# adthoms/dcora

Hardware: AMD Instinct MI355X
Metric: RBCD iterations/sec, sphere2500 5-agent split (higher is better)
Workload: dtype f64

## Files before the change

### dcora_amd/__init__.py

```python
import ctypes as C
import gzip
import os
import shutil
import tempfile

import numpy as np

from . import capi
from .capi import DcoraError, Dims, ROptParams, ROptResult, RbcdOptions, F, unF, check

__all__ = ["QuadraticProblem", "QuadraticOptimizer", "ROptParameters", "Dataset", "Csr", "RbcdSession", "RaRbcdSession", "DcoraError",
           "build_Q_pgo", "dual_certificate", "is_psd", "min_eig", "fast_verification", "manifold_project",
           "device_count"]


def device_count():
    return capi.lib().dcora_device_count()


class Csr:

    def __init__(self, n, rp, ci, v):
        self.n = int(n)
        self.rp = np.ascontiguousarray(rp, dtype=np.int32)
# ... 247 lines not shown
    def projectToTangentSpace(self, Y, V):
        out = self._out()
        check(capi.lib().dcora_problem_tangent_project(self.h, F(Y), F(V), out))
        return unF(out, self.r, self.k)

    def escapeSaddle(self, Xopt, theta, v, gradient_tolerance=1e-6, preconditioned_gradient_tolerance=1e-6,
                     isSecondOrder=False):
        out = self._out()
        ok = C.c_int()
        check(capi.lib().dcora_problem_escape_saddle(self.h, F(Xopt), float(theta),
                                                     np.ascontiguousarray(v, np.float64), gradient_tolerance,
                                                     preconditioned_gradient_tolerance, int(isSecondOrder), out,
                                                     C.byref(ok)))
        return (unF(out, self.r, self.k) if ok.value else None)

    def time_qapply(self, reps=100):
        ms, by = C.c_double(), C.c_double()
        check(capi.lib().dcora_problem_time_qapply(self.h, reps, C.byref(ms), C.byref(by)))
        return ms.value, by.value


def _time_precond(self, reps=100):
    ms, by = C.c_double(), C.c_double()
    check(capi.lib().dcora_problem_time_precond(self.h, reps, C.byref(ms), C.byref(by)))
    return ms.value, by.value


QuadraticProblem.time_precond = _time_precond


def _precond_info(self):
    info = np.zeros(5)
    check(capi.lib().dcora_problem_precond_info(self.h, info))
    return {"kind": {0: "none", 1: "dense", 2: "sparse"}[int(info[0])], "launches": int(info[1]),
            "nnzL": int(info[2]), "setup_ms": float(info[3]), "stored_doubles_per_apply": float(info[4])}


QuadraticProblem.precond_info = _precond_info


def _qapply_info(self):
    info = np.zeros(4)
    check(capi.lib().dcora_problem_qapply_info(self.h, info))
    return {"kernel": "k_spmm_bsrq" if info[0] else "k_spmm", "nnz": int(info[1]), "blocks": int(info[2]),
            "stored_matrix_bytes": float(info[3])}


QuadraticProblem.qapply_info = _qapply_info


def _solver_info(self):
    info = np.zeros(2)
    check(capi.lib().dcora_problem_solver_info(self.h, info))
    return {"tcg": {0: "three launches", 1: "two launches", 2: "one launch per run"}[int(info[0])]}


QuadraticProblem.solver_info = _solver_info


def time_qapply_rotating(problems, reps=60):
    arr = (C.c_void_p * len(problems))(*[getattr(p.h, 'value', p.h) for p in problems])
    ms = C.c_double()
    check(capi.lib().dcora_problem_time_qapply_rotating(arr, len(problems), reps, C.byref(ms)))
    return ms.value


def precond_cache_info():
    v = np.zeros(4)
    check(capi.lib().dcora_precond_cache_info(v))
    return {"hits": int(v[0]), "misses": int(v[1]), "entries": int(v[2]), "device_bytes": float(v[3])}


def precond_cache_clear():
    check(capi.lib().dcora_precond_cache_clear())


class QuadraticOptimizer:

    def __init__(self, problem, params=None):
        self.problem = problem
        self.params = params or ROptParameters()
        self.result = ROptResult()

    def optimize(self, Y):
        out = np.zeros(self.problem.r * self.problem.k)
        check(capi.lib().dcora_optimizer_optimize(self.problem.h, C.byref(self.params.c), F(Y), out,
                                                  C.byref(self.result)))
        return unF(out, self.problem.r, self.problem.k)

    def getOptResult(self):
        return self.result.as_dict()


def manifold_project(r, d, n, M, l=0, b=0, device=0, layout=0):
    dims = Dims(r, d, n, l, b, layout)
    k = (d + 1) * n + l + b
    out = np.zeros(r * k)
    check(capi.lib().dcora_manifold_project(C.byref(dims), F(M), out, device))
    return unF(out, r, k)


def dual_certificate(r, d, n, X, Q, l=0, b=0, device=0, layout=0):
    dims = Dims(r, d, n, l, b, layout)
    h = C.c_void_p()
    check(capi.lib().dcora_cert_dual_matrix(C.byref(dims), F(X), Q.rp, Q.ci, Q.v, device, C.byref(h)))
    return Csr(*capi.take_csr(h))

# ... 107 lines not shown
        self.k = (ds.d + 1) * ds.n
        o = _rbcd_options(num_robots, r, acceleration, restart_interval, params, rank, world_size, device, stream)
        dsh = ds.handle()
        self.h = C.c_void_p()
        try:
            if robust is None:
                check(capi.lib().dcora_rbcd_create(dsh, C.byref(o), C.byref(self.h)))
            else:
                fx = _fixed_flags(ds, fixed_weight)
                check(capi.lib().dcora_rbcd_create_robust(dsh, C.byref(o), C.byref(robust.c),
                                                          None if fx is None else fx.ctypes.data_as(C.c_void_p),
                                                          C.byref(self.h)))
        finally:
            capi.lib().dcora_dataset_destroy(dsh)
        self.m = ds.m

    def close(self):
        if getattr(self, "h", None):
            capi.lib().dcora_rbcd_destroy(self.h)
            self.h = None

    def __del__(self):
        try:
            self.close()
        except Exception:
            pass

    def set_X(self, X):
        check(capi.lib().dcora_rbcd_set_X(self.h, F(X)))

    def get_X(self):
        out = np.zeros(self.r * self.k)
        check(capi.lib().dcora_rbcd_get_X(self.h, out))
        return unF(out, self.r, self.k)

    def iterate(self, selected):
        c2, gn, nxt = C.c_double(), C.c_double(), C.c_int()
        bn = np.zeros(self.R)
        check(capi.lib().dcora_rbcd_iterate(self.h, selected, C.byref(c2), C.byref(gn),
                                            bn.ctypes.data_as(C.c_void_p), C.byref(nxt)))
        return c2.value, gn.value, bn, nxt.value

    def iterate_set(self, agents, allow_adjacent=False):
        a = np.ascontiguousarray(agents, dtype=np.int32)
        check(capi.lib().dcora_rbcd_iterate_set(self.h, a, a.size, int(allow_adjacent)))

    def set_acceleration(self, on):
        check(capi.lib().dcora_rbcd_set_acceleration(self.h, int(bool(on))))

    def colours(self):
        col, nc = np.zeros(self.R, np.int32), C.c_int()
        check(capi.lib().dcora_rbcd_agent_colours(self.h, col, C.byref(nc)))
        return col, nc.value

    def evaluate(self):
        c2, gn, nxt = C.c_double(), C.c_double(), C.c_int()
        bn = np.zeros(self.R)
        check(capi.lib().dcora_rbcd_evaluate(self.h, C.byref(c2), C.byref(gn), bn.ctypes.data_as(C.c_void_p),
                                             C.byref(nxt)))
        return c2.value, gn.value, bn, nxt.value

    def run(self, max_iters=1000, rgrad_tol=0.1):
        it = C.c_int()
        cost, gn = np.zeros(max_iters), np.zeros(max_iters)
        sel = np.zeros(max_iters, np.int32)
        check(capi.lib().dcora_rbcd_run(self.h, max_iters, rgrad_tol, C.byref(it), cost.ctypes.data_as(C.c_void_p),
                                        gn.ctypes.data_as(C.c_void_p), sel.ctypes.data_as(C.c_void_p)))
        n = it.value
        return dict(iters=n, cost=cost[:n], gradnorm=gn[:n], selected=sel[:n])

    def last_result(self):
        r = ROptResult()
        check(capi.lib().dcora_rbcd_last_result(self.h, C.byref(r)))
        return r.as_dict()

    def update_weights(self, reset_to_initial=False):
        c = np.zeros(3, np.int32)
        check(capi.lib().dcora_rbcd_update_weights(self.h, int(bool(reset_to_initial)), c.ctypes.data_as(C.c_void_p)))
        return {"accepted": int(c[0]), "rejected": int(c[1]), "undecided": int(c[2])}

    def set_weights(self, w):
        w = np.ascontiguousarray(w, np.float64)
        if w.shape != (self.m,):
            raise ValueError("set_weights needs one weight per measurement")
        check(capi.lib().dcora_rbcd_set_weights(self.h, w))

    def get_weights(self):
        w = np.zeros(self.m)
        check(capi.lib().dcora_rbcd_get_weights(self.h, w))
        return w

    def robust_info(self):
        mu, n = C.c_double(), C.c_int()
        check(capi.lib().dcora_rbcd_robust_info(self.h, C.byref(mu), C.byref(n)))
        return {"mu": mu.value, "updates": n.value}

    def X_device_ptr(self):
        p = C.c_void_p()
        check(capi.lib().dcora_rbcd_X_device_ptr(self.h, C.byref(p)))
        return p.value

    def public_count(self, agent):
        c = C.c_int()
        check(capi.lib().dcora_rbcd_public_count(self.h, agent, C.byref(c)))
        return c.value

# ... 284 lines not shown
```

### dcora_amd/capi.py

```python
import ctypes as C
import os
import subprocess

import numpy as np

_HERE = os.path.dirname(os.path.abspath(__file__))
LIB_PATH = os.path.join(_HERE, "lib", "libdcora_hip.so")
HEADER_PATH = os.path.join(os.path.dirname(_HERE), "include", "dcora_hip.h")


class DcoraError(RuntimeError):
    def __init__(self, status, msg):
        super().__init__("dcora status %d: %s" % (status, msg))
        self.status = status


class Dims(C.Structure):
    _fields_ = [("r", C.c_int), ("d", C.c_int), ("n", C.c_int), ("l", C.c_int), ("b", C.c_int), ("layout", C.c_int)]


LAYOUT_AUTO, LAYOUT_SE, LAYOUT_RA = 0, 1, 2


class ROptParams(C.Structure):
# ... 100 lines not shown
    "dcora_rbcd_agent_colours": (C.c_int, [_vp, _ip, _PI]),
    "dcora_rbcd_evaluate": (C.c_int, [_vp, _PD, _PD, _vp, _PI]),
    "dcora_rbcd_agent_iterate": (C.c_int, [_vp, C.c_int, C.c_int]),
    "dcora_rbcd_agent_get_X": (C.c_int, [_vp, C.c_int, _dp]),
    "dcora_rbcd_agent_set_X": (C.c_int, [_vp, C.c_int, _dp]),
    "dcora_rbcd_agent_update_neighbor": (C.c_int, [_vp, C.c_int, C.c_int, C.c_int, _ip, _dp, C.c_int]),
    "dcora_rbcd_agent_last_skipped": (C.c_int, [_vp, C.c_int, _PI]),
    "dcora_rbcd_agent_info": (C.c_int, [_vp, C.c_int, _PI, _PI, _PI]),
    "dcora_rbcd_last_result": (C.c_int, [_vp, C.POINTER(ROptResult)]),
    "dcora_rbcd_profile_tcg_runs": (C.c_int, [_vp, C.c_int]),
    "dcora_rbcd_profile_tcg_read": (C.c_int, [_vp, _dp]),
    "dcora_rbcd_create_robust": (C.c_int, [_vp, C.POINTER(RbcdOptions), C.POINTER(RobustParams), _vp, C.POINTER(_vp)]),
    "dcora_rbcd_update_weights": (C.c_int, [_vp, C.c_int, _vp]),
    "dcora_rbcd_set_weights": (C.c_int, [_vp, _dp]),
    "dcora_rbcd_get_weights": (C.c_int, [_vp, _dp]),
    "dcora_rbcd_robust_info": (C.c_int, [_vp, _PD, _PI]),
    "dcora_rbcd_create_robust_ranks": (C.c_int, [_vp, C.POINTER(RbcdOptions), C.POINTER(RobustParams), _vp, C.c_char_p,
                                                 C.POINTER(_vp), C.POINTER(_vp)]),
    "dcora_rbcd_X_device_ptr": (C.c_int, [_vp, C.POINTER(_vp)]),
    "dcora_rbcd_public_count": (C.c_int, [_vp, C.c_int, _PI]),
    "dcora_rbcd_public_indices": (C.c_int, [_vp, C.c_int, _ip]),
    "dcora_rbcd_pack_public_dev": (C.c_int, [_vp, C.c_int, _vp]),
    "dcora_rbcd_unpack_public_dev": (C.c_int, [_vp, C.c_int, _vp]),
    "dcora_rbcd_phase_nonselected": (C.c_int, [_vp, C.c_int]),
    "dcora_rbcd_phase_selected": (C.c_int, [_vp, C.c_int]),
    "dcora_rbcd_phase_evaluate_dev": (C.c_int, [_vp, _vp]),
    "dcora_rbcd_synchronize": (C.c_int, [_vp]),
    "dcora_exchange_create": (C.c_int, [_vp, C.c_char_p, C.POINTER(_vp)]),
    "dcora_exchange_destroy": (C.c_int, [_vp]),
    "dcora_exchange_create_ra": (C.c_int, [_vp, C.c_char_p, C.POINTER(_vp)]),
    "dcora_exchange_info": (C.c_int, [_vp, _dp]),
    "dcora_exchange_link_report": (C.c_int, [_vp, _dp]),
    "dcora_exchange_post": (C.c_int, [_vp, _ip, C.c_int]),
    "dcora_exchange_wait": (C.c_int, [_vp, _ip, C.c_int]),
    "dcora_exchange_evaluate": (C.c_int, [_vp, _PD, _PD, _vp, _PI]),
    "dcora_exchange_rbcd_iterate": (C.c_int, [_vp, C.c_int, _PD, _PD, _vp, _PI]),
    "dcora_exchange_rbcd_tick": (C.c_int, [_vp, _ip, C.c_int, C.c_int]),
    "dcora_exchange_set_X": (C.c_int, [_vp, _dp]),
    "dcora_exchange_gather_X": (C.c_int, [_vp, _dp]),
    "dcora_exchange_barrier": (C.c_int, [_vp]),
    "dcora_exchange_all_ready": (C.c_int, [_vp, C.c_int, _PI]),
    "dcora_exchange_update_weights": (C.c_int, [_vp, C.c_int, _vp]),
    "dcora_exchange_set_weights": (C.c_int, [_vp, _dp]),
    "dcora_exchange_get_weights": (C.c_int, [_vp, _dp]),
    "dcora_exchange_certify": (C.c_int, [_vp, C.c_int, _vp, _vp, _vp, C.c_double, _PI, _PD, _PD, _dp,
                                         C.POINTER(C.c_longlong), _PI]),
    "dcora_exchange_host_selftest": (C.c_int, [C.c_char_p, C.c_int, C.c_int, C.c_int, C.c_int, _PD]),
    "dcora_debug_exchange_leave_stale": (C.c_int, [C.c_char_p, C.c_int, C.c_int]),
    "dcora_debug_exchange_probe_fault": (C.c_int, [C.c_int]),
    "dcora_cert_prepare": (C.c_int, [C.POINTER(Dims), _ip, _ip, C.c_int, C.c_int]),
    "dcora_debug_tcg_run_fault": (C.c_int, [C.c_int]),
    "dcora_debug_tcg_run_fault_at": (C.c_int, [C.c_int, C.c_int]),
    "dcora_problem_solver_info": (C.c_int, [_vp, _dp]),
    "dcora_ra_rbcd_create": (C.c_int, [_vp, C.POINTER(RbcdOptions), C.POINTER(_vp)]),
    "dcora_ra_rbcd_destroy": (C.c_int, [_vp]),
    "dcora_ra_rbcd_info": (C.c_int, [_vp, _PI, _vp]),
    "dcora_ra_rbcd_set_X": (C.c_int, [_vp, _dp]),
    "dcora_ra_rbcd_get_X": (C.c_int, [_vp, _dp]),
    "dcora_ra_rbcd_iterate": (C.c_int, [_vp, C.c_int, _PD, _PD, _vp, _PI]),
    "dcora_ra_rbcd_evaluate": (C.c_int, [_vp, _PD, _PD, _vp, _PI]),
    "dcora_ra_rbcd_run": (C.c_int, [_vp, C.c_int, C.c_double, _PI, _vp, _vp, _vp]),
    "dcora_ra_rbcd_last_result": (C.c_int, [_vp, C.POINTER(ROptResult)]),
    "dcora_problem_time_qapply": (C.c_int, [_vp, C.c_int, _PD, _PD]),
    "dcora_problem_time_qapply_rotating": (C.c_int, [C.POINTER(_vp), C.c_int, C.c_int, _PD]),
    "dcora_problem_qapply_info": (C.c_int, [_vp, _dp]),
    "dcora_problem_time_precond": (C.c_int, [_vp, C.c_int, _PD, _PD]),
    "dcora_problem_precond_info": (C.c_int, [_vp, _dp]),
    "dcora_precond_cache_info": (C.c_int, [_dp]),
    "dcora_precond_cache_clear": (C.c_int, []),
    "dcora_robust_params_default": (None, [C.POINTER(RobustParams)]),
    "dcora_robust_weights": (C.c_int, [C.POINTER(RobustParams), C.c_int, C.c_int, _dp, _dp]),
    "dcora_chi2inv": (C.c_int, [C.c_double, C.c_int, _PD]),
    "dcora_robust_error_threshold_at_quantile": (C.c_int, [C.c_double, C.c_int, _PD]),
    "dcora_robust_single_rotation_averaging": (C.c_int, [C.c_int, C.c_int, _dp, _vp, C.c_double, _dp, _ip]),
    "dcora_robust_single_pose_averaging": (C.c_int, [C.c_int, C.c_int, _dp, _dp, _vp, _vp, C.c_double, _dp, _dp, _ip]),
    "dcora_agent_neighbor_transforms": (C.c_int, [C.c_int, C.c_int, _ip, _dp, _dp, _dp, _dp, _dp]),
    "dcora_agent_robust_neighbor_transform": (C.c_int, [C.c_int, C.c_int, _dp, C.c_int, C.c_int, _dp, _PI, _PI]),
    "dcora_log_trajectory": (C.c_int, [C.c_char_p, C.c_int, C.c_int, _dp]),
    "dcora_fixed_stiefel_variable": (C.c_int, [C.c_int, C.c_int, _dp]),
    "dcora_agent_initialize_in_global_frame": (C.c_int, [C.POINTER(Dims), _dp, _dp, _dp, _dp]),
    "dcora_measurement_errors": (C.c_int, [_vp, C.c_int, _dp, _dp, C.c_int]),
    "dcora_solve_pgo": (C.c_int, [_vp, C.POINTER(ROptParams), _vp, _dp, C.POINTER(ROptResult), C.c_int]),
    "dcora_solve_robust_pgo": (C.c_int, [_vp, C.POINTER(ROptParams), C.POINTER(RobustParams), _vp, _vp, _dp, _vp,
                                         C.c_int]),
    "dcora_round_align_trajectory": (C.c_int, [C.POINTER(Dims), _dp, _vp, C.c_int, _dp, _vp, _vp, C.c_int]),
    "dcora_round_project_solution_raslam": (C.c_int, [C.POINTER(Dims), _dp, _dp, C.c_int]),
}

_lib = None


def lib():
    global _lib
    if _lib is None:
        if not os.path.exists(LIB_PATH):
            raise DcoraError(-1, "libdcora_hip.so is not built (run __graft_entry__.build()); there is no fallback")
        L = C.CDLL(LIB_PATH)
        for name, (res, args) in SIGNATURES.items():
            fn = getattr(L, name)
            fn.restype = res
            fn.argtypes = args
        _lib = L
    return _lib


def check(status):
# ... 23 lines not shown
```

### dcora_amd/csrc/capi.hip

```cpp
#include <cstdio>
#include <cstring>
#include <new>

#include "../../include/dcora_hip.h"
#include "cert.h"
#include "device_chol.h"
#include "device_problem.h"
#include "host_graph.h"
#include "host_threads.h"
#include "ra_rbcd.h"
#include "rbcd.h"
#include "precond_cache.h"
#include "exchange.h"
#include "host_robust.h"
#include "robust.h"
#include "round.h"

namespace dcora {
const std::string &get_last_error();
}
using namespace dcora;

struct dcora_problem_s {
  DeviceProblem p;
// ... 192 lines not shown
int dcora_problem_time_qapply(dcora_problem_t p, int reps, double *avg_ms, double *bytes) {
  return abi_call({p, avg_ms, bytes}, [&] { return p->p.time_qapply(reps, avg_ms, bytes); });
}

int dcora_problem_time_qapply_rotating(const dcora_problem_t *ps, int count, int reps, double *avg_ms) {
  return abi_call({ps, avg_ms}, [&]() -> int {
    if (count < 1) return bad("null");
    for (int i = 0; i < count; ++i)
      if (!ps[i]) return bad("null problem");
    DeviceProblem &P0 = ps[0]->p;
    DCORA_HIP(hipSetDevice(P0.device));
    std::vector<hipStream_t> keep(count);
    for (int i = 0; i < count; ++i) {
      DCORA_HIP(hipStreamSynchronize(ps[i]->p.st));
      keep[i] = ps[i]->p.st;
      ps[i]->p.st = P0.st;
    }
    hipEvent_t e0, e1;
    DCORA_HIP(hipEventCreate(&e0));
    DCORA_HIP(hipEventCreate(&e1));
    for (int i = 0; i < count; ++i) ps[i]->p.enqueue_egrad(ps[i]->p.X0.p, ps[i]->p.EG0.p, nullptr);
    DCORA_HIP(hipEventRecord(e0, P0.st));
    for (int i = 0; i < reps; ++i) {
      DeviceProblem &P = ps[i % count]->p;
      P.enqueue_egrad(P.X0.p, P.EG0.p, nullptr);
    }
    DCORA_HIP(hipEventRecord(e1, P0.st));
    DCORA_HIP(hipEventSynchronize(e1));
    float ms = 0;
    DCORA_HIP(hipEventElapsedTime(&ms, e0, e1));
    (void)hipEventDestroy(e0);
    (void)hipEventDestroy(e1);
    for (int i = 0; i < count; ++i) ps[i]->p.st = keep[i];
    *avg_ms = (double)ms / reps;
    return DCORA_OK;
  });
}
int dcora_problem_qapply_info(dcora_problem_t p, double *info) {
  return abi_call({p, info}, [&]() -> int {
    const DeviceProblem &P = p->p;
    info[0] = P.has_bsr ? 1 : 0;
    info[1] = (double)P.Q.nnz;
    info[2] = P.has_bsr ? (double)P.Qb.nblocks : 0.0;
    info[3] = P.has_bsr ? P.Qb.nblocks * (8.0 * (P.m.d + 1) * (P.m.d + 1) + 4.0) + 4.0 * (P.m.n + 1)
                        : 12.0 * P.Q.nnz + 4.0 * (P.m.k + 1);
    return DCORA_OK;
  });
}

int dcora_problem_solver_info(dcora_problem_t p, double *info) {
  return abi_call({p, info}, [&]() -> int {
    const DeviceProblem &P = p->p;
    info[0] = !P.use_pc() ? 0 : (P.tcg_run_ok ? 2 : 1);
    return DCORA_OK;
  });
}
int dcora_debug_tcg_run_fault(int runs) {
  g_tcg_run_fault_skip.store(0);
  g_tcg_run_fault.store(runs < 0 ? 0 : runs);
  return DCORA_OK;
}
int dcora_debug_tcg_run_fault_at(int skip, int runs) {
  g_tcg_run_fault_skip.store(skip < 0 ? 0 : skip);
  g_tcg_run_fault.store(runs < 0 ? 0 : runs);
  return DCORA_OK;
}
int dcora_problem_time_precond(dcora_problem_t p, int reps, double *avg_ms, double *bytes) {
  return abi_call({p, avg_ms, bytes}, [&] { return p->p.time_precond(reps, avg_ms, bytes); });
}
int dcora_problem_precond_info(dcora_problem_t p, double *info) {
  return abi_call({p, info}, [&]() -> int {
    const DeviceProblem &P = p->p;
    info[0] = !P.has_precond ? 0 : (P.sparse_precond ? 2 : 1);
    info[1] = !P.has_precond ? 0 : (P.sparse_precond ? P.sp.launches() : 1);
    info[2] = (double)P.precond_nnzL;
    info[3] = P.precond_setup_ms;
    info[4] = !P.has_precond ? 0 : (P.sparse_precond ? P.sp.weights_per_apply : (double)P.m.k * P.m.k);
    return DCORA_OK;
  });
}

int dcora_debug_sparse_weights_digest(dcora_problem_t p, double *out4) {
  return abi_call({p, out4}, [&]() -> int {
    const DeviceProblem &P = p->p;
    if (!P.sparse_precond || !P.sp.im) return bad("the problem has no sparse preconditioner");
    const DevBuf<double> &v = P.sp.im->vals;
    std::vector<double> h(v.n);
    DCORA_HIP(hipSetDevice(P.device));
    DCORA_HIP(hipMemcpy(h.data(), v.p, v.n * sizeof(double), hipMemcpyDeviceToHost));
    long double s0 = 0, s1 = 0, s2 = 0;
    for (size_t i = 0; i < h.size(); ++i) {
      s0 += h[i];
      s1 += std::fabs(h[i]);
      s2 += h[i] * (double)(i % 97 + 1);
    }
    out4[0] = (double)h.size();
    out4[1] = (double)s0;
    out4[2] = (double)s1;
    out4[3] = (double)s2;
    return DCORA_OK;
  });
}

}

namespace {
// ... 675 lines not shown
    const int rc = local_robust_session(s, "dcora_exchange_set_weights");
    return rc ? rc : s->s.set_weights(w);
  });
}
int dcora_rbcd_get_weights(dcora_rbcd_t s, double *w) {
  return abi_call({s, w}, [&] {
    const int rc = robust_session(s);
    return rc ? rc : s->s.get_weights(w);
  });
}
int dcora_rbcd_robust_info(dcora_rbcd_t s, double *mu, int *updates) {
  return abi_call({s}, [&] {
    const int rc = robust_session(s);
    if (rc) return rc;
    if (mu) *mu = s->s.robust->cost.mu();
    if (updates) *updates = s->s.robust->updates;
    return (int)DCORA_OK;
  });
}
int dcora_rbcd_destroy(dcora_rbcd_t s) {
  delete s;
  return DCORA_OK;
}
int dcora_rbcd_set_X(dcora_rbcd_t s, const double *X) {
  return abi_call({s, X}, [&] { return s->s.set_X(X); });
}
int dcora_rbcd_get_X(dcora_rbcd_t s, double *X) {
  return abi_call({s, X}, [&] { return s->s.get_X(X); });
}
int dcora_rbcd_iterate(dcora_rbcd_t s, int selected, double *cost2, double *gradnorm, double *block_norms,
                       int *next_selected) {
  return abi_call({s}, [&] { return s->s.iterate(selected, cost2, gradnorm, block_norms, next_selected); });
}
int dcora_rbcd_run(dcora_rbcd_t s, int max_iters, double rgrad_tol, int *iters_done, double *cost2_trace,
                   double *gradnorm_trace, int *selected_trace) {
  return abi_call({s}, [&] {
    return run_passes(s->s, max_iters, rgrad_tol, iters_done, cost2_trace, gradnorm_trace, selected_trace);
  });
}
int dcora_rbcd_iterate_set(dcora_rbcd_t s, const int *set, int count, int allow_adjacent) {
  return abi_call({s}, [&] {
    return count > 0 && !set ? bad("null argument") : s->s.iterate_set(set, count, allow_adjacent);
  });
}
int dcora_rbcd_set_acceleration(dcora_rbcd_t s, int acceleration) {
  return abi_call({s}, [&] { return s->s.set_acceleration(acceleration != 0); });
}
int dcora_rbcd_agent_colours(dcora_rbcd_t s, int *colours, int *ncolours) {
  return abi_call({s, colours}, [&] { return s->s.agent_colours(colours, ncolours); });
}
int dcora_rbcd_evaluate(dcora_rbcd_t s, double *cost2, double *gradnorm, double *block_norms, int *next_selected) {
  return abi_call({s}, [&] { return s->s.evaluate_central(cost2, gradnorm, block_norms, next_selected); });
}
int dcora_rbcd_agent_iterate(dcora_rbcd_t s, int agent, int do_optimization) {
  return abi_call({s}, [&] { return s->s.agent_iterate(agent, do_optimization != 0); });
}
int dcora_rbcd_agent_update_neighbor(dcora_rbcd_t s, int agent, int neighbor, int count, const int *frames,
                                     const double *poses, int auxiliary) {
  return abi_call({s}, [&] {
    if (count > 0 && (!frames || !poses)) return bad("null argument");
    return s->s.agent_update_neighbor(agent, neighbor, count, frames, poses, auxiliary != 0);
  });
}
namespace {
bool agent_ok(dcora_rbcd_t s, int agent) { return agent >= 0 && agent < s->s.R; }
}
int dcora_rbcd_agent_last_skipped(dcora_rbcd_t s, int agent, int *skipped) {
  return abi_call({s, skipped}, [&] {
    if (!agent_ok(s, agent)) return bad("bad agent");
    *skipped = s->s.agents[agent].last_skipped ? 1 : 0;
    return (int)DCORA_OK;
  });
}
int dcora_rbcd_agent_get_X(dcora_rbcd_t s, int agent, double *X) {
  return abi_call({s, X}, [&] { return s->s.agent_get_X(agent, X); });
}
int dcora_rbcd_agent_set_X(dcora_rbcd_t s, int agent, const double *X) {
  return abi_call({s, X}, [&] { return s->s.agent_set_X(agent, X); });
}
int dcora_rbcd_agent_info(dcora_rbcd_t s, int agent, int *num_poses, int *first_pose, int *iteration_number) {
  return abi_call({s}, [&] {
    if (!agent_ok(s, agent)) return bad("bad agent");
    const AgentDev &a = s->s.agents[agent];
    if (num_poses) *num_poses = a.n;
    if (first_pose) *first_pose = a.col0 / (s->s.d + 1);
    if (iteration_number)
      *iteration_number = (int)s->s.agent_it.size() == s->s.R ? s->s.agent_it[agent] : s->s.iteration;
    return (int)DCORA_OK;
  });
}
int dcora_rbcd_last_result(dcora_rbcd_t s, dcora_ropt_result *res) {
  return abi_call({s, res}, [&] { return s->s.last_result(res); });
}
int dcora_rbcd_X_device_ptr(dcora_rbcd_t s, double **X_dev) {
  return abi_call({s, X_dev}, [&] {
    *X_dev = s->s.Xg.p;
    return DCORA_OK;
  });
}
int dcora_rbcd_public_count(dcora_rbcd_t s, int agent, int *count) {
  return abi_call({s, count}, [&] {
    if (!agent_ok(s, agent)) return bad("bad agent");
    *count = (int)s->s.agents[agent].public_poses.size();
    return (int)DCORA_OK;
  });
}
// ... 540 lines not shown
```

### dcora_amd/csrc/device_problem.h

```cpp
#pragma once
#include <hip/hip_runtime.h>

#include <functional>
#include <memory>
#include <string>
#include <vector>

#include "../../include/dcora_hip.h"
#include "host_sparse.h"
#include "kernels.h"
#include "sparse_precond.h"

namespace dcora {

void set_last_error(const std::string &s);
int hip_fail(hipError_t e, const char *what, const char *file, int line);
#define DCORA_HIP(call)                                                        \
  do {                                                                         \
    hipError_t e_ = (call);                                                    \
    if (e_ != hipSuccess) return ::dcora::hip_fail(e_, #call, __FILE__, __LINE__); \
  } while (0)

template <class T>
struct DevBuf {
// ... 130 lines not shown
  bool foldable() const { return im && im->nhub == 0 && im->in_pos.p != nullptr; }
  SpFold fold() const {
    SpFold f;
    if (foldable()) {
      f.y = y.p;
      f.in_pos = im->in_pos.p;
      f.out_pos = im->out_pos.p;
    }
    return f;
  }
  SpFold fold_generic() const;
  int attach(std::shared_ptr<const SpImage> image, int rcap);
  int launches() const { return (int)im->levels.size() + 2; }
  void apply(hipStream_t st, int r, Buf2 R, double *Z, Gate g, bool levels_only = false,
             const std::function<bool()> *after_first = nullptr) const;
  double bytes_per_apply(int r) const;
};

int stream_acquire(int device, hipStream_t *out);
void stream_release(int device, hipStream_t st);
int host_flags_acquire(HostFlags **host, HostFlags **dev, int *slot);
void host_flags_release(HostFlags *host, int slot);

int precond_prebuild_dense(const std::vector<const HostCsr *> &Qs, double reg, int block, int device);

class DeviceProblem {
 public:
  ManiDesc m{};
  int device = 0;
  hipStream_t st = nullptr;
  bool own_stream = false;
  DevCsr Q;
  DevBsr Qb;
  bool has_bsr = false;
  int enq_qapply(Buf2 X, int selX, const double *Gp, Buf2 Y, int selY, double *partials, Gate g);
  DevBuf<double> G;
  bool has_G = false;
  DevBuf<double> Minv;
  int ldm = 0;
  SparsePrecond sp;
  std::shared_ptr<const DevBuf<double>> Minv_shared;
  bool precond_cache_hit = false;
  bool sparse_precond = false;
  bool has_precond = false;
  double precond_setup_ms = 0;
  long precond_nnzL = 0;

  DevBuf<double> X0, X1, EG0, EG1, RG0, RG1, S0, S1;
  DevBuf<double> delta, eta, Heta, res, z, Hd, W, Zt;
  DevBuf<double> delta2, res2, Zpart;
  bool tcg_run_ok = false;
  bool concurrent_solves = false;
  DevBuf<unsigned> tcg_sync;
  bool profile_tcg_runs = false;
  std::vector<hipEvent_t> run_events;
  size_t run_events_used = 0;
  int profile_tcg_read(double *launches, double *total_us);
  bool fused = false;
  bool group = false;
  DevBuf<double> pA, pB, pC, p1, p2, p3, scal;
  DevBuf<SolverCtl> ctl;
  DevBuf<double> arena;
  int hf_slot = -1;
  HostFlags *hf = nullptr;
  HostFlags *hf_dev = nullptr;
  std::vector<double> stage;

  long nelem() const { return (long)m.r * m.k; }
  Buf2 Xb() const { return Buf2{{X0.p, X1.p}}; }
  Buf2 EGb() const { return Buf2{{EG0.p, EG1.p}}; }
  Buf2 RGb() const { return Buf2{{RG0.p, RG1.p}}; }
  Buf2 Sb() const { return Buf2{{S0.p, S1.p}}; }

  ~DeviceProblem();
  int init(const dcora_dims &dims, const HostCsr &Qh, const double *Gh, double reg, int device_, hipStream_t shared);
  int set_G_host(const double *Gh);
  int build_preconditioner(const HostCsr &Qh, double reg);
  int set_values(const HostCsr &Q_on_pattern, hipStream_t stream, std::vector<double> *stage);

  int npA() const { return has_bsr ? spmm_bsr_grid(m.n) : spmm_grid(m.k, m.r) + Q.n_long; }
  int npPose() const { return pose_grid(m); }
  int enq_rgrad(Buf2 X, Buf2 EG, Buf2 RG, Buf2 S, int sel, double *partials, Gate g, double *posenorm = nullptr);
  int enq_retract(Buf2 X, const double *V, double alpha, Buf2 out, int selOut, Buf2 grad, const double *HV,
                  double *partials, Gate g);
  int npVec() const { return vec_grid(nelem()); }
  void enqueue_egrad(const double *X, double *EG, double *partials);
  void enqueue_precond(const double *X, const double *V, double *out);
  void enq_minv(Buf2 R, double *Z, const double *p2, int np2, Gate g);

  int cost(const double *Xh, double *f);
  int eucgrad(const double *Xh, double *out);
  int riegrad(const double *Xh, double *out, double *norm);
  int hessvec(const double *Xh, const double *Vh, double *out);
  int hessvec_solver_form(const double *Xh, const double *Vh, double *out, double *dots);
  bool hess_one_launch() const;
  int precondition(const double *Xh, const double *Vh, double *out);
  int retract(const double *Xh, const double *Vh, double *out);
  int tangent_project(const double *Xh, const double *Vh, double *out);
  int optimize(const dcora_ropt_params &prm, const double *X0h, double *Xout, dcora_ropt_result *res);
  int escape_saddle(const double *Xopt, double theta, const double *v, double gtol, double pgtol, bool second_order,
                    double *Xout, int *success);

  int optimize_dev(const dcora_ropt_params &prm);
  int fetch_result(dcora_ropt_result *res);
  Buf2 result_pick(const SolverCtl **c) const;
  int result(double **X);
// ... 23 lines not shown
```

### dcora_amd/csrc/device_problem.hip

```cpp
#include <atomic>

#include "device_problem.h"
#include "env.h"
#include "device_chol.h"
#include "host_threads.h"
#include "precond_cache.h"

#include <algorithm>
#include <chrono>
#include <cmath>
#include <cstdio>
#include <cstdlib>
#include <cstring>
#include <map>
#include <mutex>

namespace dcora {

static thread_local std::string g_last_error;
void set_last_error(const std::string &s) { g_last_error = s; }
const std::string &get_last_error() { return g_last_error; }
int hip_fail(hipError_t e, const char *what, const char *file, int line) {
  char buf[512];
  std::snprintf(buf, sizeof buf, "HIP error %d (%s) at %s:%d in %s", (int)e, hipGetErrorString(e), file, line, what);
// ... 165 lines not shown
  DCORA_HIP(hipSetDevice(device));
  if (shared) {
    st = shared;
    own_stream = false;
  } else {
    const int rcs = stream_acquire(device, &st);
    if (rcs) return rcs;
    own_stream = true;
  }
  lap("stream");
  int rc = Q.upload(Qh);
  if (rc) return rc;
  lap("Q upload");
  const bool want_bsr = m.n >= 8192;
  if (m.se && m.r <= 8 && m.n > 0 && want_bsr && !env::generic_solver()) {
    rc = Qb.upload(bsr_from_csr(Qh, m.d + 1));
    if (rc) return rc;
    has_bsr = true;
  }
  const size_t N = (size_t)nelem();
  const size_t NS = (size_t)m.n * m.d * m.d + m.l + 1;
  fused = fused_supported(m) && Qh.nnz() > 0 && !env::generic_solver();
  group = group_supported(m) && !env::generic_solver();
  {
    struct Slot {
      DevBuf<double> *b;
      size_t n;
    };
    std::vector<Slot> slots;
    for (DevBuf<double> *b : {&G, &X0, &X1, &EG0, &EG1, &RG0, &RG1, &delta, &eta, &Heta, &res, &z, &Hd, &W, &Zt})
      slots.push_back({b, N});
    slots.push_back({&delta2, N});
    if (fused) {
      slots.push_back({&res2, N});
      slots.push_back({&Zpart, (size_t)fused_nsplit(m) * N});
    }
    slots.push_back({&S0, NS});
    slots.push_back({&S1, NS});
    for (DevBuf<double> *b : {&pB, &pC, &p1, &p2, &p3}) slots.push_back({b, (size_t)4 * kMaxPartials});
    slots.push_back({&pA, 2 * (size_t)kBsrMaxGrid});
    slots.push_back({&scal, 64});
    auto pad = [](size_t n) { return (n + 31) & ~(size_t)31; };
    size_t total = 0;
    for (const Slot &sl : slots) total += pad(sl.n);
    DCORA_HIP(arena.alloc(total));
    DCORA_HIP(hipMemsetAsync(arena.p, 0, total * sizeof(double), st));
    size_t off = 0;
    for (const Slot &sl : slots) {
      sl.b->borrow(arena.p + off, sl.n);
      off += pad(sl.n);
    }
  }
  DCORA_HIP(ctl.alloc(1));
  {
    const int rc2 = host_flags_acquire(&hf, &hf_dev, &hf_slot);
    if (rc2) return rc2;
  }
  DCORA_HIP(hipStreamSynchronize(st));
  lap("workspace");
  if (Gh) {
    rc = set_G_host(Gh);
    if (rc) return rc;
  }
  if (reg >= 0) {
    rc = build_preconditioner(Qh, reg);
    if (rc) return rc;
  }
  lap("precond");
  if (fused && has_precond && !sparse_precond && !has_bsr && Q.n_long == 0 && env::solver_tcg() >= 0) {
    hipDeviceProp_t prop;
    DCORA_HIP(hipGetDeviceProperties(&prop, device));
    tcg_run_ok = tcg_run_supported(m, ldm, prop.multiProcessorCount, tcg_run_max_rows_nnz(m, Qh.rp.data()));
    if (tcg_run_ok) {
      DCORA_HIP(tcg_sync.alloc((size_t)tcg_run_sync_words()));
      DCORA_HIP(hipMemsetAsync(tcg_sync.p, 0, sizeof(unsigned) * (size_t)tcg_run_sync_words(), st));
    }
  }
  return DCORA_OK;
}

int DeviceProblem::set_values(const HostCsr &Q_on_pattern, hipStream_t stream, std::vector<double> *stage) {
  const int rc = Q.set_values(Q_on_pattern, stream);
  if (rc || !has_bsr) return rc;
  *stage = std::move(bsr_from_csr(Q_on_pattern, m.d + 1).bv);
  if (stage->size() != Qb.bv.n) {
    set_last_error("set_values: the matrix does not have the uploaded pattern");
    return DCORA_ERR_BAD_ARG;
  }
  DCORA_HIP(hipMemcpyAsync(Qb.bv.p, stage->data(), sizeof(double) * stage->size(), hipMemcpyHostToDevice, stream));
  return DCORA_OK;
}

int DeviceProblem::set_G_host(const double *Gh) {
  DCORA_HIP(hipSetDevice(device));
  if (Gh) {
    DCORA_HIP(hipMemcpy(G.p, Gh, (size_t)nelem() * sizeof(double), hipMemcpyHostToDevice));
    has_G = true;
  } else {
    DCORA_HIP(hipMemset(G.p, 0, (size_t)nelem() * sizeof(double)));
    has_G = false;
  }
  return DCORA_OK;
}

int precond_prebuild_dense(const std::vector<const HostCsr *> &Qs, double reg, int block, int device) {
  if (env::precond_mode() == 2 || env::factor_on_host() || env::precond_cache_mb() <= 0) return DCORA_OK;
// ... 446 lines not shown
      if (std::chrono::duration<double>(std::chrono::steady_clock::now() - t0).count() > timeout_s) return false;
    }
#if defined(__x86_64__)
    __builtin_ia32_pause();
#endif
  }
  return true;
}
}

int DeviceProblem::profile_tcg_read(double *launches, double *total_us) {
  DCORA_HIP(hipSetDevice(device));
  DCORA_HIP(hipStreamSynchronize(st));
  double us = 0;
  for (size_t i = 0; i + 1 < run_events_used; i += 2) {
    float ms = 0;
    if (hipEventElapsedTime(&ms, run_events[i], run_events[i + 1]) == hipSuccess) us += 1e3 * ms;
  }
  *launches = (double)(run_events_used / 2);
  *total_us = us;
  run_events_used = 0;
  return DCORA_OK;
}

bool DeviceProblem::use_pc() const {
  const int forced = env::solver_bc();
  if (sparse_precond || !has_precond) return false;
  if (forced < 0) return false;
  if (!forced && !fused_pc_preferred(m, ldm)) return false;
  return fused_pc_ready(m, ldm);
}

struct DeviceProblem::RtrForm {
  DeviceProblem &p;
  TcgForm form;
  int &seq;
  const int solve_first;
  SolverCtl *const c;
  const CsrDev Qv;
  const BsrDev Qbv;
  const double *const Gp;
  const long N;
  const int nA, nP, nV, nPB;
  const bool sparse;
  const SpFold sfg;
  const bool hess_fused;
  const int nPG;
  const double *const Mi;
  const bool folded;
  const SpFold sf;
  const int nsl;
  const int nZ;
  const bool gf, gfb;
  unsigned *const sync_p;
  const int nsync;
  double *const dbuf[2];
  double *const rbuf[2];

  RtrForm(DeviceProblem &p_, TcgForm f, int &seq_)
      : p(p_), form(f), seq(seq_), solve_first(seq_ + 1), c(p.ctl.p), Qv(p.Q.view()),
        Qbv(p.has_bsr ? p.Qb.view() : BsrDev{}), Gp(p.has_G ? p.G.p : nullptr), N(p.nelem()), nA(p.npA()),
        nP(p.npPose()), nV(p.npVec()), nPB(fused_pose_blocks(p.m)), sparse(p.sparse_precond),
        sfg(f == TcgForm::generic && sparse ? p.sp.fold_generic() : SpFold()),
        hess_fused(f == TcgForm::generic && p.hess_one_launch()),
        nPG(sparse ? fused_update_grid(p.m) : fused_precond_grid(p.m)), Mi(sparse ? nullptr : p.Minv.p),
        folded(sparse && p.sp.foldable()), sf(folded ? p.sp.fold() : SpFold{}), nsl(sparse ? 1 : -1),
        nZ(f == TcgForm::pc || f == TcgForm::run ? fused_pc_blocks(p.m) : nPB),
        gf(f != TcgForm::generic && !p.has_bsr && p.Q.n_long == 0), gfb(f != TcgForm::generic && p.has_bsr),
        sync_p(f == TcgForm::run ? p.tcg_sync.p : nullptr), nsync(f == TcgForm::run ? tcg_run_sync_words() : 0),
        dbuf{p.delta.p, p.delta2.p}, rbuf{p.res.p, p.res2.p} {}

  bool outer_done() const { return p.hf->outer_done_seq >= solve_first; }
  bool stopped(int tcg_first) const { return p.hf->tcg_done_seq >= tcg_first || outer_done(); }
  int nAe() const { return gf ? nPB : nA; }

  int eval(int sel) {
    const auto g = [&] {
      ++seq;
      return sel ? Gate{c, seq, 1} : Gate{};
    };
    const Buf2 kNoBuf{{nullptr, nullptr}};
    if (form == TcgForm::generic) {
      p.enq_qapply(p.Xb(), sel, Gp, p.EGb(), sel, p.pA.p, g());
      launch_rgrad(p.st, p.m, p.Xb(), p.EGb(), p.RGb(), p.Sb(), sel, p.pB.p, g());
      return nP;
    }
    if (gf) return launch_fused_grad(p.st, p.m, Qv, p.Xb(), Gp, p.EGb(), p.RGb(), p.Sb(), sel, p.pA.p, p.pB.p, nullptr, g());
    if (gfb)
      return launch_fused_grad_bsr(p.st, p.m.r, p.m.d, Qbv, p.Xb(), Gp, kNoBuf, p.RGb(), p.Sb(), sel, p.pA.p, p.pB.p,
                                   nullptr, g());
    p.enq_qapply(p.Xb(), sel, Gp, p.EGb(), sel, p.pA.p, g());
    return p.enq_rgrad(p.Xb(), p.EGb(), p.RGb(), p.Sb(), sel, p.pB.p, g());
  }

  int first() {
    switch (form) {
      case TcgForm::generic: {
        launch_tcg_begin(p.st, N, p.RGb(), p.eta.p, p.Heta.p, p.res.p, c, ++seq);
        const int s = seq;
        p.enq_minv(buf1(p.res.p), p.Zt.p, nullptr, 0, Gate{c, ++seq, 1});
        launch_tangent(p.st, p.m, p.Xb(), p.Zt.p, p.z.p, p.res.p, p.p3.p, nullptr, 0, c, p.hf_dev, ++seq, 1, 0);
        return s;
      }
      case TcgForm::run: {
        const int s = launch_run();
        if (s != 0) return s;
        p.tcg_run_ok = false;
        form = TcgForm::pc;
      }
        [[fallthrough]];
      case TcgForm::pc:
        if (launch_fused_pc(p.st, p.m, p.ldm, Mi, p.RGb(), p.Xb(), nullptr, nullptr, p.eta.p, p.Heta.p, nullptr, rbuf[0],
                            p.z.p, nullptr, 0, p.p3.p, c, p.hf_dev, ++seq, 0, 1) < 0) {
          set_last_error("k_fused_pc could not be launched on this device");
          return -1;
        }
        return seq;
      case TcgForm::split:
        launch_fused_precond(p.st, p.m, p.ldm, Mi, p.RGb(), nullptr, nullptr, p.eta.p, p.Heta.p, nullptr, rbuf[0],
                             p.Zpart.p, nullptr, 0, p.p2.p, c, p.hf_dev, ++seq, 0, 1, sf);
        return seq;
    }
    return -1;
  }
  int launch_run() {
    hipEvent_t e1 = nullptr;
    if (p.profile_tcg_runs) {
      while (p.run_events.size() < p.run_events_used + 2) {
        hipEvent_t e = nullptr;
        if (hipEventCreate(&e) != hipSuccess) {
          set_last_error("hipEventCreate failed (k_tcg_run profile)");
          return -1;
        }
        p.run_events.push_back(e);
      }
      (void)hipEventRecord(p.run_events[p.run_events_used], p.st);
      e1 = p.run_events[p.run_events_used + 1];
      p.run_events_used += 2;
    }
    if (launch_tcg_run(p.st, p.m, p.ldm, Mi, Qv, p.RGb(), p.Xb(), p.Sb(), dbuf[0], dbuf[1], p.Hd.p, p.eta.p, p.Heta.p,
// ... 75 lines not shown

  int trial() {
    switch (form) {
      case TcgForm::generic:
        launch_retract(p.st, p.m, p.Xb(), p.eta.p, 1.0, p.Xb(), 1, p.RGb(), p.Heta.p, p.pC.p, Gate{c, ++seq, 1});
        return nP;
      case TcgForm::split:
        return p.enq_retract(p.Xb(), p.eta.p, 1.0, p.Xb(), 1, p.RGb(), p.Heta.p, p.pC.p, Gate{c, ++seq, 1});
      default:
        return nZ;
    }
  }
};

int DeviceProblem::rtr_dev(const dcora_ropt_params &prm, TcgForm form) {
  constexpr int kLookahead = 2;
  const auto t0 = std::chrono::steady_clock::now();
  t0_ms_ = std::chrono::duration<double, std::milli>(t0.time_since_epoch()).count();
  const bool single = (prm.RTR_iterations == 1);
  const int max_outer = single ? 12 : prm.RTR_iterations;
  const int max_inner = prm.RTR_tCG_iterations;
  if (seq_ > 1500000000) {
    DCORA_HIP(hipStreamSynchronize(st));
    hf->last_seq_done = 0;
    hf->tcg_done_seq = 0;
    hf->outer_done_seq = 0;
    hf->go_seq = 0;
    hf->reject_seq = 0;
    seq_ = 0;
  }
  int &seq = seq_;
  RtrForm f(*this, form, seq);
  CtlInit ci;
  ci.enable = 1;
  ci.tol = prm.gradnorm_tol;
  ci.Delta = prm.RTR_initial_radius;
  ci.maxDelta = single ? prm.RTR_initial_radius : 5 * prm.RTR_initial_radius;
  ci.max_outer = max_outer;
  ci.stop_on_accept = single ? 1 : 0;
  ci.max_inner = max_inner;
  auto timed_out = [&]() {
    set_last_error("rtr_dev: device did not make progress (spin timeout)");
    return DCORA_ERR_HIP;
  };
  auto first_failed = [&]() -> int {
    DCORA_HIP(hipStreamSynchronize(st));
    return DCORA_ERR_HIP;
  };
  auto time_is_up = [&]() {
    return std::chrono::duration<double>(std::chrono::steady_clock::now() - t0).count() > 5.0;
  };
  auto run_gave_up = [&]() { return f.form == TcgForm::run && hf->tcg_abort_seq >= f.solve_first; };

  int nG = f.eval(0);
  launch_rtr_init(st, pA.p, f.nAe(), pB.p, nG, f.c, hf_dev, ++seq, ci, f.sync_p, f.nsync);
  int last_pace_seq = seq;
  std::vector<int> last_seq((size_t)std::max(1, max_inner));
  int next_first_seq = time_is_up() ? 0 : f.first();
  int last_run_seq = 0;
  for (int outer = 0; outer < max_outer || (f.form == TcgForm::run && last_run_seq > 0); ++outer) {
    const bool tail = outer >= max_outer;
    if (!tail && next_first_seq < 0) return first_failed();
    const int need_seq = tail ? last_run_seq : last_pace_seq;
    if (!spin_until([&] { return hf->last_seq_done >= need_seq || f.outer_done() || run_gave_up(); }, 20.0))
      return timed_out();
    if (tail && !run_gave_up()) break;
    if (run_gave_up()) {
      DCORA_HIP(hipStreamSynchronize(st));
      const int armed = INT_MAX;
      DCORA_HIP(hipMemcpy(&f.c->outer_done_stamp, &armed, sizeof(int), hipMemcpyHostToDevice));
      if (hf->last_seq_done < last_pace_seq) --outer;
      hf->tcg_abort_seq = 0;
      tcg_run_ok = false;
      f.form = TcgForm::pc;
      next_first_seq = f.first();
      if (next_first_seq < 0) return first_failed();
    }
    if (f.outer_done()) break;
    if (next_first_seq == 0) break;
    const int tcg_first_seq = next_first_seq;
    last_run_seq = f.form == TcgForm::run ? tcg_first_seq : 0;
    f.rest(outer > 0 && hf->reject_seq == last_pace_seq);
    for (int j = 0; j < max_inner && f.form != TcgForm::run; ++j) {
      if (j >= kLookahead) {
        const int need = last_seq[j - kLookahead];
        if (!spin_until([&] { return hf->last_seq_done >= need || f.stopped(tcg_first_seq); }, 20.0))
          return timed_out();
      }
      if (hf->tcg_done_seq >= tcg_first_seq) break;
      const int go = f.tcg_iter(j, max_inner, tcg_first_seq);
      if (go < 0) return timed_out();
      if (go == 0) break;
      last_seq[j] = seq;
    }
    const int nR = f.trial();
    nG = f.eval(1);
    launch_rtr_decide(st, pA.p, f.nAe(), pB.p, nG, pC.p, nR, f.c, hf_dev, ++seq, f.sync_p, f.nsync);
    last_pace_seq = seq;
    if (outer + 1 < max_outer) next_first_seq = time_is_up() ? 0 : f.first();
  }
  pending_ = true;
  return DCORA_OK;
}

int DeviceProblem::escape_saddle(const double *Xopt, double theta, const double *v, double gtol, double pgtol,
                                 bool second_order, double *Xout, int *success) {
  if (!has_precond) {
    set_last_error("escapeSaddle needs the preconditioner");
    return DCORA_ERR_NO_PRECONDITIONER;
  }
  DCORA_HIP(hipSetDevice(device));
  const int r = m.r, k = m.k;
  std::vector<double> Xp((size_t)r * k, 0.0), Xd((size_t)r * k, 0.0);
  for (int j = 0; j < k; ++j) {
    for (int t = 0; t < r - 1; ++t) Xp[(size_t)j * r + t] = Xopt[(size_t)j * (r - 1) + t];
    Xd[(size_t)j * r + (r - 1)] = v[j];
  }
  int rc = upload(Xp.data(), X0.p, nelem());
  if (rc) return rc;
  rc = upload(Xd.data(), eta.p, nelem());
  if (rc) return rc;
  DCORA_HIP(hipStreamSynchronize(st));
  double FX = 0;
  rc = eval_dev(X0.p, &FX, nullptr);
  if (rc) return rc;
  const double alpha_min = 1e-6;
  double alpha = second_order ? std::max(16 * alpha_min, 100 * gtol / std::fabs(theta)) : 1.0;
  std::vector<double> alphas, fvals;
  *success = 0;
  while (alpha >= alpha_min) {
    launch_retract(st, m, buf1(X0.p), eta.p, alpha, buf1(X1.p), 0, buf1(RG0.p), nullptr, nullptr, Gate{});
    enqueue_egrad(X1.p, EG1.p, pA.p);
    launch_rgrad(st, m, buf1(X1.p), buf1(EG1.p), buf1(RG1.p), buf1(S1.p), 0, pB.p, Gate{});
    enqueue_precond(X1.p, RG1.p, z.p);
    launch_dot(st, nelem(), z.p, z.p, p3.p);
    launch_sum_partials(st, pA.p, npA(), 2, 2, scal.p);
    launch_sum_partials(st, pB.p, npPose(), 1, 1, scal.p + 2);
    launch_sum_partials(st, p3.p, npVec(), 1, 1, scal.p + 3);
    double s[4];
    rc = download(scal.p, s, 4);
    if (rc) return rc;
    const double FXt = 0.5 * s[0] + s[1], gn = std::sqrt(s[2]), pgn = std::sqrt(s[3]);
    alphas.push_back(alpha);
    fvals.push_back(FXt);
    if (FXt < FX && gn > gtol && pgn > pgtol) {
      *success = 1;
      return download(X1.p, Xout, nelem());
    }
    alpha /= 2;
  }
// ... 81 lines not shown
```

### dcora_amd/csrc/env.cpp

```cpp
#include "env.h"

#include <cstdlib>
#include <cstring>

namespace dcora {
namespace env {
namespace {
bool is(const char *name, const char *value) {
  const char *e = std::getenv(name);
  return e && std::strcmp(e, value) == 0;
}
}

bool init_timing() {
  static const bool v = std::getenv("DCORA_INIT_TIMING") != nullptr;
  return v;
}
int precond_mode() {
  return is("DCORA_PRECOND", "dense") ? 1 : is("DCORA_PRECOND", "sparse") ? 2 : 0;
}
bool generic_solver() {
  return is("DCORA_SOLVER", "generic");
}
int solver_tcg() {
  return is("DCORA_SOLVER_TCG", "launch") ? -1 : is("DCORA_SOLVER_TCG", "run") ? 1 : 0;
}
int solver_bc() {
  static const int v = is("DCORA_SOLVER_BC", "pc") ? 1 : is("DCORA_SOLVER_BC", "split") ? -1 : 0;
  return v;
}
bool factor_on_host() {
  static const bool v = is("DCORA_FACTOR", "host");
  return v;
}
bool fill_on_host() {
  static const bool v = is("DCORA_SP_FILL", "host");
  return v;
}
bool lanczos_sync() {
  static const bool v = is("DCORA_LANCZOS", "sync");
  return v;
}
int host_threads() {
  static const int v = [] {
    const char *e = std::getenv("DCORA_HOST_THREADS");
    return e ? (std::atoi(e) > 0 ? std::atoi(e) : 1) : 0;
  }();
  return v;
}
double precond_cache_mb() {
  static const double v = [] {
    const char *e = std::getenv("DCORA_PRECOND_CACHE_MB");
    return e ? std::atof(e) : 8192.0;
  }();
  return v;
}
const char *exchange() {
  static const char *v = std::getenv("DCORA_EXCHANGE");
  return v;
}
const char *exchange_wait() {
  static const char *v = std::getenv("DCORA_EXCHANGE_WAIT");
  return v;
}
double exchange_timeout_s() {
  static const double v = [] {
    const char *e = std::getenv("DCORA_EXCHANGE_TIMEOUT_S");
    const double x = e ? std::atof(e) : 0.0;
    return x > 0 ? x : 120.0;
  }();
  return v;
}

}
}
```

### dcora_amd/csrc/env.h

```cpp
#pragma once

namespace dcora {
namespace env {

bool init_timing();
int precond_mode();
bool generic_solver();
int solver_tcg();
int solver_bc();
bool factor_on_host();
bool fill_on_host();
bool lanczos_sync();
int host_threads();
double precond_cache_mb();
const char *exchange();
const char *exchange_wait();
double exchange_timeout_s();

}
}
```

### dcora_amd/csrc/kernels.h

```cpp
#pragma once
#include <hip/hip_runtime.h>

#include <atomic>
#include <climits>
#include <vector>

namespace dcora {

constexpr int kMaxPartials = 1024;
constexpr int kBsrMaxGrid = 4096;
constexpr int kBlock = 256;

struct ManiDesc {
  int r, d, n, l, b, k, se;
  __host__ __device__ int rot_col(int i) const { return se ? i * (d + 1) : i * d; }
  __host__ __device__ int sphere_col(int i) const { return d * n + i; }
  __host__ __device__ int num_euc() const { return se ? n : n + b; }
  __host__ __device__ int euc_col(int e) const { return se ? e * (d + 1) + d : d * n + l + e; }
};
inline ManiDesc make_mani(int r, int d, int n, int l, int b, int layout = 0) {
  ManiDesc m;
  m.r = r; m.d = d; m.n = n; m.l = l; m.b = b;
  m.se = (layout == 2) ? 0 : ((l == 0 && b == 0) ? 1 : 0);
  m.k = (d + 1) * n + l + b;
// ... 61 lines not shown
struct Gate {
  const SolverCtl *ctl = nullptr;
  int seq = 0;
  int gate = 0;
};

int spmm_grid(int nrows, int r);
int spmm_dir_fix_grid(const ManiDesc &m, int nrows);
int launch_spmm_dir_fix(hipStream_t st, const ManiDesc &m, const CsrDev &A, Buf2 X, Buf2 Sblk, const double *z,
                        const double *d_old, double *d_new, double *Hd, const double *p3, int np3, double *p1,
                        SolverCtl *ctl, int seq, int iter);
void launch_spmm_dir(hipStream_t st, int r, const CsrDev &A, const double *z, const double *d_old, double *d_new,
                     double *W, const double *p3, int np3, SolverCtl *ctl, int seq, int iter);
inline int spmm_slots(const CsrDev &A, int r) { return spmm_grid(A.nrows, r) + A.n_long; }
void launch_spmm(hipStream_t st, int r, const CsrDev &A, Buf2 X, int selX, const double *G, Buf2 Y, int selY,
                 double *partials, Gate g);

int spmm_bsr_grid(int nbrows);
void launch_spmm_bsr(hipStream_t st, int r, int d, const BsrDev &A, Buf2 X, int selX, const double *G, Buf2 Y,
                     int selY, double *partials, Gate g);

int pose_grid(const ManiDesc &m);
void launch_rgrad(hipStream_t st, const ManiDesc &m, Buf2 X, Buf2 EG, Buf2 RG, Buf2 Sblk, int sel,
                  double *partials, Gate g);
struct SpFold {
  double *y = nullptr;
  const int *in_pos = nullptr, *out_pos = nullptr;
  int h = 0;
  const int *hub_idx = nullptr;
  const double *hub_U = nullptr, *hub_x2 = nullptr;
};
void launch_tangent(hipStream_t st, const ManiDesc &m, Buf2 X, const double *V, double *out, const double *R,
                    double *partials, const double *p2, int np2, SolverCtl *ctl, HostFlags *hf, int seq,
                    int gate, int iter, SpFold sf = SpFold());
void launch_hessfix(hipStream_t st, const ManiDesc &m, Buf2 X, Buf2 Sblk, const double *V, const double *W,
                    double *HV, double *partials, Gate g);
void launch_retract(hipStream_t st, const ManiDesc &m, Buf2 X, const double *V, double alpha, Buf2 out,
                    int selOut, Buf2 grad, const double *HV, double *partials, Gate g);
void launch_polar(hipStream_t st, const ManiDesc &m, double c0, const double *A, double c1, const double *B,
                  double c2, const double *C, double *out);

void launch_nesterov(hipStream_t st, const ManiDesc &m, int mode, int restart, int skip_lo, int skip_hi, double alpha,
                     double gamma, double *X, double *V, double *Y, double *XPrev, double *Yloc,
                     const double *Xloc);

void launch_dense_apply(hipStream_t st, int r, int k, int ldm, const double *Minv, Buf2 R, double *Z,
                        const double *p2, int np2, Gate g);

int vec_grid(long nelem);
struct CtlInit {
  int enable = 0;
  double tol = 0, Delta = 0, maxDelta = 0;
  int max_outer = 0, stop_on_accept = 0, max_inner = 0;
};
void launch_rtr_init(hipStream_t st, const double *pA, int npA, const double *pB, int npB, SolverCtl *ctl,
                     HostFlags *hf, int seq, CtlInit ci = CtlInit(), unsigned *tcg_sync = nullptr, int nsync = 0);
void launch_tcg_begin(hipStream_t st, long nelem, Buf2 grad, double *eta, double *Heta, double *res,
                      SolverCtl *ctl, int seq);
void launch_tcg_update1(hipStream_t st, long nelem, const double *delta, const double *Hd, double *eta,
                        double *Heta, double *res, const double *p1, int np1, double *p2, SolverCtl *ctl,
                        HostFlags *hf, int seq, int iter, int r = 1, SpFold sf = SpFold());
void launch_tcg_update2(hipStream_t st, long nelem, const double *z, double *delta, const double *p3, int np3,
                        SolverCtl *ctl, HostFlags *hf, int seq, int iter);
void launch_rtr_decide(hipStream_t st, const double *pA, int npA, const double *pB, int npB, const double *pC,
                       int npC, SolverCtl *ctl, HostFlags *hf, int seq, unsigned *tcg_sync = nullptr, int nsync = 0);

void launch_axpby(hipStream_t st, long nelem, double a, const double *x, double b, const double *y, double *out);
void launch_sum_partials(hipStream_t st, const double *partials, int np, int stride, int count, double *out);
void launch_dot(hipStream_t st, long nelem, const double *x, const double *y, double *partials);
void launch_gather_cols(hipStream_t st, int r, int ncols, const int *src_col, const double *X, double *out);
void launch_scatter_cols(hipStream_t st, int r, int ncols, const int *dst_col, const double *in, double *X);
void launch_block_dots(hipStream_t st, int r, int nagents, const int *col_start, const double *A, const double *B,
                       double *out);

void launch_lambda_blocks(hipStream_t st, const ManiDesc &m, const double *X, const double *XQ, double *Lblk);
void launch_lanczos_proj(hipStream_t st, int n, int nv, const double *V, const double *w, double *partials);
void launch_lanczos_sub(hipStream_t st, int n, int nv, const double *V, const double *h, double *w);
constexpr int kLanczosFuseParts = 256;
void launch_lanczos_sub_sum(hipStream_t st, int n, int nv, const double *V, const double *partials, int npart,
                            double *hout, double *w, double *dotpart);
void launch_lanczos_keep(hipStream_t st, int nv, const double *h, double *hout);
constexpr double kLanczosDead = 1e-10;
void launch_lanczos_next(hipStream_t st, int n, const double *partials, int npart, double *beta_out, int *flag,
                         const double *w, double *vnext, const double *hrow, int nv);
void launch_scale_shift(hipStream_t st, int n, double shift, const double *x, double *y);
void launch_scale(hipStream_t st, int n, const double *alpha_dev_inv_sqrt ,
                  const double *w, double *out);

bool fused_supported(const ManiDesc &m);
bool group_supported(const ManiDesc &m);
int fused_pose_blocks(const ManiDesc &m);
int fused_nsplit(const ManiDesc &m);
int fused_precond_grid(const ManiDesc &m);
int fused_update_grid(const ManiDesc &m);
int launch_fused_hess(hipStream_t st, const ManiDesc &m, const CsrDev &Q, const double *z, const double *d_old,
                       double *d_new, Buf2 X, Buf2 S, double *Hd, const double *p3, int np3, double *p1,
                       SolverCtl *ctl, int seq, int iter,
                      const BsrDev *Ab = nullptr );
void launch_fused_precond(hipStream_t st, const ManiDesc &m, int ldm, const double *Minv, Buf2 grad,
                          const double *delta, const double *Hd, double *eta, double *Heta, const double *res_old,
                          double *res_new, double *Zpart, const double *p1, int np1, double *p2, SolverCtl *ctl,
                          HostFlags *hf, int seq, int iter, int first, SpFold sf = SpFold());
int fused_pc_blocks(const ManiDesc &m);
bool tcg_run_supported(const ManiDesc &m, int ldm, int cus, int max_rows_nnz);
int tcg_run_sync_words();
extern std::atomic<int> g_tcg_run_fault;
extern std::atomic<int> g_tcg_run_fault_skip;
int tcg_run_max_rows_nnz(const ManiDesc &m, const int *rowptr);
int launch_tcg_run(hipStream_t st, const ManiDesc &m, int ldm, const double *Minv, const CsrDev &Q, Buf2 grad, Buf2 X,
                   Buf2 S, double *d0, double *d1, double *Hd, double *eta, double *Heta, double *z, double *p1r,
                   double *p3, double *pC, unsigned *sync, SolverCtl *ctl, HostFlags *hf, int seq);
bool fused_pc_preferred(const ManiDesc &m, int ldm);
bool fused_pc_ready(const ManiDesc &m, int ldm);
int launch_fused_pc(hipStream_t st, const ManiDesc &m, int ldm, const double *Minv, Buf2 grad, Buf2 X,
                    const double *delta, const double *Hd, double *eta, double *Heta, const double *res_old,
                    double *res_new, double *z, const double *p1, int np1, double *p3, SolverCtl *ctl, HostFlags *hf,
                    int seq, int iter, int first, double *pC = nullptr );
void launch_fused_finish(hipStream_t st, const ManiDesc &m, Buf2 X, const double *Zpart, const double *res,
                         double *z, const double *p2, int np2, double *p3, SolverCtl *ctl, HostFlags *hf, int seq,
                         int iter, int first, int nsplit = -1 , SpFold sf = SpFold(),
                         double *zraw = nullptr );
int launch_fused_grad_bsr(hipStream_t st, int r, int d, const BsrDev &A, Buf2 X, const double *G, Buf2 EG, Buf2 RG, Buf2 S,
                          int sel, double *pA, double *pB, double *posenorm, Gate g,
                          const int *agent_start = nullptr, int agents = 0, int *wg_per_agent = nullptr);
int launch_fused_grad(hipStream_t st, const ManiDesc &m, const CsrDev &Q, Buf2 X, const double *G, Buf2 EG, Buf2 RG,
                      Buf2 Sblk, int sel, double *pA, double *pB, double *posenorm, Gate g);
int launch_g_rgrad(hipStream_t st, const ManiDesc &m, Buf2 X, Buf2 EG, Buf2 RG, Buf2 Sblk, int sel, double *partials,
                   double *posenorm, Gate g);
void launch_ctl_init(hipStream_t st, SolverCtl *c, double tol, double Delta, double maxDelta, int max_outer,
                     int stop_on_accept, int max_inner);
void launch_eval_finish(hipStream_t st, int R, const int *pose_start, const double *posenorm, const double *pA,
                        int npA, EvalOut *out_dev, int seq, double *split_scratch = nullptr, int nposes = 0,
                        const double *agent_partials = nullptr, int wg_per_agent = 0);
int eval_split_doubles();
int launch_g_retract(hipStream_t st, const ManiDesc &m, Buf2 X, const double *V, double alpha, Buf2 out, int selOut,
                     Buf2 grad, const double *HV, double *partials, Gate g);
void launch_g_nesterov(hipStream_t st, const ManiDesc &m, int mode, int restart, int skip_lo, int skip_hi,
                       double alpha, double gamma, double *X, double *V, double *Y, double *XPrev, double *Yloc,
                       Buf2 Xloc, const SolverCtl *ctl, double *inner_Yloc = nullptr);

#if defined(__HIPCC__)
template <int CTRL>
__device__ __forceinline__ double dpp_move(double v) {
  int lo = __double2loint(v), hi = __double2hiint(v);
  lo = __builtin_amdgcn_update_dpp(0, lo, CTRL, 0xF, 0xF, true);
  hi = __builtin_amdgcn_update_dpp(0, hi, CTRL, 0xF, 0xF, true);
  return __hiloint2double(hi, lo);
}
__device__ __forceinline__ double readlane_f64(double v, int lane) {
  const int lo = __builtin_amdgcn_readlane(__double2loint(v), lane);
  const int hi = __builtin_amdgcn_readlane(__double2hiint(v), lane);
  return __hiloint2double(hi, lo);
}
__device__ __forceinline__ double wave_sum_dpp(double v) {
  v += dpp_move<0xB1>(v);
  v += dpp_move<0x4E>(v);
  v += dpp_move<0x141>(v);
  v += dpp_move<0x140>(v);
  return (readlane_f64(v, 0) + readlane_f64(v, 16)) + (readlane_f64(v, 32) + readlane_f64(v, 48));
}
__device__ __forceinline__ double wave_sum(double v) { return wave_sum_dpp(v); }
__device__ __forceinline__ double block_sum(double v, double *sm) {
  v = wave_sum(v);
  const int w = threadIdx.x >> 6, nw = (blockDim.x + 63) >> 6;
  __syncthreads();
  if ((threadIdx.x & 63) == 0) sm[w] = v;
  __syncthreads();
  double t = 0;
  for (int i = 0; i < nw; ++i) t += sm[i];
  return t;
}
__device__ __forceinline__ double sum_partials(const double *p, int np, int stride, int off, double *sm) {
  double v = 0;
  for (int i = threadIdx.x; i < np; i += blockDim.x) v += p[(size_t)i * stride + off];
  return block_sum(v, sm);
}
__device__ __forceinline__ void host_store(volatile int *p, int v) {
  __hip_atomic_store(const_cast<int *>(p), v, __ATOMIC_RELAXED, __HIP_MEMORY_SCOPE_SYSTEM);
}
// ... 31 lines not shown
```

### dcora_amd/csrc/kernels.hip

```cpp
#include "kernels.h"
#include "tcg_rules.h"

namespace dcora {

template <int N>
__device__ __forceinline__ void sum_partials_n(const double *const (&p)[N], const int (&np)[N], const int (&st)[N],
                                               const int (&off)[N], double *sm, double (&out)[N]) {
  double v[N];
#pragma unroll
  for (int q = 0; q < N; ++q) v[q] = ((int)threadIdx.x < np[q]) ? p[q][(size_t)threadIdx.x * st[q] + off[q]] : 0.0;
#pragma unroll
  for (int q = 0; q < N; ++q)
    for (int i = threadIdx.x + blockDim.x; i < np[q]; i += blockDim.x) v[q] += p[q][(size_t)i * st[q] + off[q]];
#pragma unroll
  for (int q = 0; q < N; ++q) v[q] = wave_sum(v[q]);
  const int w = threadIdx.x >> 6, nw = (blockDim.x + 63) >> 6;
  __syncthreads();
  if ((threadIdx.x & 63) == 0)
#pragma unroll
    for (int q = 0; q < N; ++q) sm[q * 4 + w] = v[q];
  __syncthreads();
#pragma unroll
  for (int q = 0; q < N; ++q) {
    double t = 0;
    for (int i = 0; i < nw; ++i) t += sm[q * 4 + i];
    out[q] = t;
  }
}

int vec_grid(long nelem) {
  long g = (nelem + kBlock - 1) / kBlock;
  if (g < 1) g = 1;
  if (g > kMaxPartials) g = kMaxPartials;
  return (int)g;
}

constexpr int kSpmmTile = 1536;

int spmm_grid(int nrows, int r) {
  const int RB = kBlock / r;
  long nrb = (nrows + RB - 1) / RB;
  if (nrb < 1) nrb = 1;
  if (nrb > kMaxPartials) nrb = kMaxPartials;
  return (int)nrb;
}

template <bool DOTS>
__global__ __launch_bounds__(kBlock) void k_spmm(int r, CsrDev A, Buf2 Xb, int selX, const double *__restrict__ G,
                                                 Buf2 Yb, int selY, double *__restrict__ partials, Gate g,
                                                 int main_grid) {
  if (gated(g.ctl, g.seq, g.gate)) return;
  __shared__ int s_ci[kSpmmTile];
  __shared__ double s_v[kSpmmTile];
  __shared__ double s_red[16];
  const double *__restrict__ X = pick(Xb, g.ctl, selX);
  double *__restrict__ Y = pick(Yb, g.ctl, selY);
  const int RB = kBlock / r;
  const int nrb = (A.nrows + RB - 1) / RB;
  const int lj = threadIdx.x / r, t = threadIdx.x - lj * r;
  double d0 = 0, d1 = 0;
  if ((int)blockIdx.x >= main_grid) {
    const int li = ((int)blockIdx.x - main_grid) / kLongSplit, sl = ((int)blockIdx.x - main_grid) % kLongSplit;
    const int j = A.long_rows[li];
    const int rb0 = A.rp[j], re0 = A.rp[j + 1];
    const int per = (re0 - rb0 + kLongSplit - 1) / kLongSplit;
    const int pb = rb0 + sl * per, pe = min(re0, pb + per);
    double acc = 0;
    if (lj < RB) {
      for (int p = pb + lj; p < pe; p += 8 * RB) {
        int c8[8];
        double w8[8], x8[8];
#pragma unroll
        for (int q = 0; q < 8; ++q) {
          const int pp = p + q * RB;
          const bool ok = pp < pe;
          c8[q] = A.ci[ok ? pp : rb0];
          w8[q] = ok ? A.v[pp] : 0.0;
        }
#pragma unroll
        for (int q = 0; q < 8; ++q) x8[q] = X[(size_t)c8[q] * r + t];
#pragma unroll
// ... 1265 lines not shown
#pragma unroll
  for (int a = 0; a < RW; ++a)
#pragma unroll
    for (int t = 0; t < RM; ++t) acc[a][t] = 0;
  const double *rows[RW];
#pragma unroll
  for (int a = 0; a < RW; ++a) rows[a] = Minv + (size_t)min(j0 + a, k - 1) * ldm;
  for (int c = 2 * lane; c < k; c += 128) {
    const bool two = (c + 1 < k);
    double m0[RW], m1[RW];
#pragma unroll
    for (int a = 0; a < RW; ++a) {
      const double2 mm = *reinterpret_cast<const double2 *>(rows[a] + c);
      m0[a] = mm.x;
      m1[a] = two ? mm.y : 0.0;
    }
    const double *rc = R + (size_t)c * r;
#pragma unroll
    for (int t = 0; t < RM; ++t)
      if (t < r) {
        const double x0 = rc[t];
        const double x1 = two ? rc[r + t] : 0.0;
#pragma unroll
        for (int a = 0; a < RW; ++a) acc[a][t] += x0 * m0[a] + x1 * m1[a];
      }
  }
#pragma unroll
  for (int a = 0; a < RW; ++a)
#pragma unroll
    for (int t = 0; t < RM; ++t)
      if (t < r) {
        const double s = wave_sum(acc[a][t]);
        if (lane == 0 && j0 + a < k) Z[(size_t)(j0 + a) * r + t] = s;
      }
}

void launch_dense_apply(hipStream_t st, int r, int k, int ldm, const double *Minv, Buf2 R, double *Z,
                        const double *p2, int np2, Gate g) {
  constexpr int RW = 2;
  const int rows_per_block = (kBlock / 64) * RW;
  const int grid = (k + rows_per_block - 1) / rows_per_block;
  if (r <= 4)
    hipLaunchKernelGGL((k_dense_apply<4, RW>), dim3(grid), dim3(kBlock), 0, st, r, k, ldm, Minv, R, Z, p2, np2, g);
  else if (r <= 8)
    hipLaunchKernelGGL((k_dense_apply<8, RW>), dim3(grid), dim3(kBlock), 0, st, r, k, ldm, Minv, R, Z, p2, np2, g);
  else
    hipLaunchKernelGGL((k_dense_apply<16, RW>), dim3(grid), dim3(kBlock), 0, st, r, k, ldm, Minv, R, Z, p2, np2, g);
}

__global__ __launch_bounds__(kBlock) void k_rtr_init(const double *pA, int npA, const double *pB, int npB,
                                                     SolverCtl *ctl, HostFlags *hf, int seq, CtlInit ci,
                                                     unsigned *tcg_sync, int nsync) {
  __shared__ double s_red[16];
  for (int i = threadIdx.x; i < nsync; i += kBlock) tcg_sync[i] = 0u;
  if (ci.enable && threadIdx.x == 0) ctl_arm(ctl, ci);
  const double *const ps[3] = {pA, pA, pB};
  const int nps[3] = {npA, npA, npB}, sts[3] = {2, 2, 1}, offs[3] = {0, 1, 0};
  double sums[3];
  sum_partials_n<3>(ps, nps, sts, offs, s_red, sums);
  const double fq = sums[0], fg = sums[1], g2 = sums[2];
  if (threadIdx.x == 0) {
    ctl->f1 = 0.5 * fq + fg;
    ctl->ngf = sqrt(g2);
    ctl->fInit = ctl->f1;
    ctl->gradNormInit = ctl->ngf;
    if (ctl->ngf < ctl->tol || ctl->max_outer <= 0) {
      ctl->outer_done_stamp = seq;
      host_store(&hf->outer_done_seq, seq);
    }
    host_store(&hf->last_seq_done, seq);
  }
}

__global__ __launch_bounds__(kBlock) void k_tcg_begin(long nelem, Buf2 gradb, double *__restrict__ eta,
                                                      double *__restrict__ Heta, double *__restrict__ res,
                                                      SolverCtl *ctl, int seq) {
  if (gated(ctl, seq, 1)) return;
  const double *grad = pick(gradb, ctl, 0);
  for (long i = (long)blockIdx.x * kBlock + threadIdx.x; i < nelem; i += (long)gridDim.x * kBlock) {
    eta[i] = 0;
    Heta[i] = 0;
    res[i] = grad[i];
  }
  if (blockIdx.x == 0 && threadIdx.x == 0) tcg_begin_run(ctl, ctl->ngf);
}
__global__ __launch_bounds__(kBlock) void k_tcg_update1(long nelem, const double *__restrict__ delta,
                                                        const double *__restrict__ Hd, double *__restrict__ eta,
                                                        double *__restrict__ Heta, double *__restrict__ res,
                                                        const double *__restrict__ p1, int np1,
                                                        double *__restrict__ p2, SolverCtl *ctl, HostFlags *hf,
                                                        int seq, int iter, int r, SpFold sf) {
  __shared__ double s_red[16];
  const int par = iter & 1;
  const long i0 = (long)blockIdx.x * kBlock + threadIdx.x;
  const bool in0 = i0 < nelem;
  const GateWords gw = gate_words(ctl);
  double pv = ((int)threadIdx.x < np1) ? p1[threadIdx.x] : 0.0;
  const double z_r = ctl->z_r[par], d_Pd = ctl->d_Pd[par], e_Pe = ctl->e_Pe[par], e_Pd = ctl->e_Pd[par];
  const double Delta = ctl->Delta;
  double h0 = 0, dl0 = 0, et0 = 0, he0 = 0, rs0 = 0;
  int jp0 = -1;
  const long col0 = in0 ? i0 / r : 0;
  if (in0) {
    h0 = Hd[i0];
    dl0 = delta[i0];
    et0 = eta[i0];
    he0 = Heta[i0];
    rs0 = res[i0];
    if (sf.y) jp0 = sf.in_pos[col0];
  }
  asm volatile("" ::"v"(pv), "v"(h0), "v"(dl0), "v"(et0), "v"(he0), "v"(rs0), "v"(jp0), "s"(gw.outer), "s"(gw.tcg));
  if (gated(gw, ctl, seq, 2)) return;
  for (int i = threadIdx.x + blockDim.x; i < np1; i += blockDim.x) pv += p1[i];
  const double d_Hd = block_sum(pv, s_red);
  const double alpha = tcg_alpha(z_r, d_Hd);
  const double e_Pe_new = tcg_e_Pe_new(alpha, d_Pd, e_Pe, e_Pd);
  const bool boundary = tcg_boundary(d_Hd, e_Pe_new, Delta);
  const double step = boundary ? tcg_tau(d_Pd, e_Pe, e_Pd, Delta) : alpha;
  if (!boundary && blockIdx.x == 0 && threadIdx.x == 0) host_store(&hf->go_seq, seq);
  double acc = 0;
  if (in0) {
    eta[i0] = et0 + step * dl0;
    Heta[i0] = he0 + step * h0;
    if (!boundary) {
      const double rr = rs0 + alpha * h0;
      res[i0] = rr;
      acc += rr * rr;
      if (sf.y && jp0 >= 0) sf.y[(size_t)jp0 * r + (i0 - col0 * r)] = rr;
    }
  }
  for (long i = i0 + (long)gridDim.x * kBlock; i < nelem; i += (long)gridDim.x * kBlock) {
    const double h = Hd[i];
    eta[i] += step * delta[i];
    Heta[i] += step * h;
    if (!boundary) {
      const double rr = res[i] + alpha * h;
      res[i] = rr;
      acc += rr * rr;
      if (sf.y) {
        const long col = i / r;
        const int jp = sf.in_pos[col];
        if (jp >= 0) sf.y[(size_t)jp * r + (i - col * r)] = rr;
      }
    }
  }
  const double tot = block_sum(acc, s_red);
  if (threadIdx.x == 0) p2[blockIdx.x] = tot;
  if (blockIdx.x == 0 && threadIdx.x == 0) {
    ctl->alpha = alpha;
    ctl->e_Pe_n = e_Pe_new;
    if (boundary) tcg_end_run(ctl, hf, seq, tcg_boundary_status(d_Hd), iter + 1);
  }
}

__global__ __launch_bounds__(kBlock) void k_tcg_update2(long nelem, const double *__restrict__ z,
                                                        double *__restrict__ delta, const double *__restrict__ p3,
                                                        int np3, SolverCtl *ctl, HostFlags *hf, int seq, int iter) {
  if (gated(ctl, seq, 2)) return;
  __shared__ double s_red[16];
  const int par = iter & 1;
  const double z_r_new = sum_partials(p3, np3, 1, 0, s_red);
  const double beta = tcg_beta(z_r_new, ctl->z_r[par]);
  for (long i = (long)blockIdx.x * kBlock + threadIdx.x; i < nelem; i += (long)gridDim.x * kBlock)
    delta[i] = -z[i] + beta * delta[i];
  if (blockIdx.x == 0 && threadIdx.x == 0) {
    tcg_put_dir(ctl, par ^ 1, tcg_dir_next(z_r_new, beta, ctl->alpha, ctl->d_Pd[par], ctl->e_Pd[par]), ctl->e_Pe_n);
    if (iter + 1 >= ctl->max_inner) tcg_end_run_at_cap(ctl, hf, seq, iter + 1);
    host_store(&hf->last_seq_done, seq);
  }
}

__global__ __launch_bounds__(kBlock) void k_rtr_decide(const double *pA, int npA, const double *pB, int npB,
                                                       const double *pC, int npC, SolverCtl *ctl, HostFlags *hf,
                                                       int seq, unsigned *tcg_sync, int nsync) {
  if (gated(ctl, seq, 1)) return;
  __shared__ double s_red[20];
  for (int i = threadIdx.x; i < nsync; i += kBlock) tcg_sync[i] = 0u;
  const double *const ps[5] = {pA, pA, pB, pC, pC};
  const int nps[5] = {npA, npA, npB, npC, npC}, sts[5] = {2, 2, 1, 2, 2}, offs[5] = {0, 1, 0, 0, 1};
  double sums[5];
  sum_partials_n<5>(ps, nps, sts, offs, s_red, sums);
  const double fq = sums[0], fg = sums[1], g2 = sums[2], eg = sums[3], eh = sums[4];
  if (threadIdx.x == 0) {
    const double f2 = 0.5 * fq + fg;
    const double rho = (ctl->f1 - f2) / (-(eg + 0.5 * eh));
    ctl->f2 = f2;
    ctl->rho = rho;
    if (rho > 0.75) {
      if (ctl->tcg_status == TR_NEGCURVTURE || ctl->tcg_status == TR_EXCREGION) ctl->Delta = fmin(2.0 * ctl->Delta, ctl->maxDelta);
    } else if (rho < 0.25) {
      ctl->Delta *= 0.25;
    }
    const bool accept = (rho > 0.1) && isfinite(rho);
    if (accept) {
      ctl->cur ^= 1;
      ctl->f1 = f2;
      ctl->ngf = sqrt(g2);
      ctl->accepted += 1;
      ctl->last_accepted = 1;
    } else {
      ctl->last_accepted = 0;
      host_store(&hf->reject_seq, seq);
    }
    ctl->outer_it += 1;
    if (ctl->ngf < ctl->tol || ctl->outer_it >= ctl->max_outer || (ctl->stop_on_accept && accept)) {
      ctl->outer_done_stamp = seq;
      host_store(&hf->outer_done_seq, seq);
    }
    host_store(&hf->last_seq_done, seq);
  }
}

void launch_rtr_init(hipStream_t st, const double *pA, int npA, const double *pB, int npB, SolverCtl *ctl,
                     HostFlags *hf, int seq, CtlInit ci, unsigned *tcg_sync, int nsync) {
  hipLaunchKernelGGL(k_rtr_init, dim3(1), dim3(kBlock), 0, st, pA, npA, pB, npB, ctl, hf, seq, ci, tcg_sync, nsync);
}
void launch_tcg_begin(hipStream_t st, long nelem, Buf2 grad, double *eta, double *Heta, double *res,
                      SolverCtl *ctl, int seq) {
  hipLaunchKernelGGL(k_tcg_begin, dim3(vec_grid(nelem)), dim3(kBlock), 0, st, nelem, grad, eta, Heta, res, ctl,
                     seq);
}
void launch_tcg_update1(hipStream_t st, long nelem, const double *delta, const double *Hd, double *eta,
                        double *Heta, double *res, const double *p1, int np1, double *p2, SolverCtl *ctl,
                        HostFlags *hf, int seq, int iter, int r, SpFold sf) {
  hipLaunchKernelGGL(k_tcg_update1, dim3(vec_grid(nelem)), dim3(kBlock), 0, st, nelem, delta, Hd, eta, Heta, res,
                     p1, np1, p2, ctl, hf, seq, iter, r, sf);
}
void launch_tcg_update2(hipStream_t st, long nelem, const double *z, double *delta, const double *p3, int np3,
                        SolverCtl *ctl, HostFlags *hf, int seq, int iter) {
  hipLaunchKernelGGL(k_tcg_update2, dim3(vec_grid(nelem)), dim3(kBlock), 0, st, nelem, z, delta, p3, np3, ctl, hf,
                     seq, iter);
}
void launch_rtr_decide(hipStream_t st, const double *pA, int npA, const double *pB, int npB, const double *pC,
                       int npC, SolverCtl *ctl, HostFlags *hf, int seq, unsigned *tcg_sync, int nsync) {
  hipLaunchKernelGGL(k_rtr_decide, dim3(1), dim3(kBlock), 0, st, pA, npA, pB, npB, pC, npC, ctl, hf, seq, tcg_sync,
                     nsync);
}

__global__ __launch_bounds__(kBlock) void k_axpby(long nelem, double a, const double *__restrict__ x, double b,
                                                  const double *__restrict__ y, double *__restrict__ out) {
  for (long i = (long)blockIdx.x * kBlock + threadIdx.x; i < nelem; i += (long)gridDim.x * kBlock)
    out[i] = a * x[i] + (y ? b * y[i] : 0.0);
}
void launch_axpby(hipStream_t st, long nelem, double a, const double *x, double b, const double *y, double *out) {
  hipLaunchKernelGGL(k_axpby, dim3(vec_grid(nelem)), dim3(kBlock), 0, st, nelem, a, x, b, y, out);
}

__global__ __launch_bounds__(kBlock) void k_sum_partials(const double *partials, int np, int stride, int count,
                                                         double *out) {
  __shared__ double s_red[16];
  for (int c = 0; c < count; ++c) {
    const double s = sum_partials(partials, np, stride, c, s_red);
    if (threadIdx.x == 0) out[c] = s;
  }
}
void launch_sum_partials(hipStream_t st, const double *partials, int np, int stride, int count, double *out) {
  hipLaunchKernelGGL(k_sum_partials, dim3(1), dim3(kBlock), 0, st, partials, np, stride, count, out);
}

__global__ __launch_bounds__(kBlock) void k_dot(long nelem, const double *__restrict__ x,
                                                const double *__restrict__ y, double *__restrict__ partials) {
  __shared__ double s_red[16];
  double acc = 0;
// ... 177 lines not shown
```

### dcora_amd/csrc/rbcd.h

```cpp
#pragma once
#include <chrono>
#include <functional>
#include <memory>
#include <string>
#include <vector>

#include "device_problem.h"
#include "exchange_session.h"
#include "host_graph.h"
#include "host_robust.h"
#include "robust.h"

namespace dcora {

struct AgentDev {
  int id = 0, n = 0, col0 = 0;
  bool hosted = false;
  bool v_feasible = false;
  std::unique_ptr<DeviceProblem> prob;
  DevCsr coupling;
  std::vector<int> public_poses;
  DevBuf<int> public_cols;
  std::vector<int> neighbors;
  hipStream_t own = nullptr;
// ... 11 lines not shown
  dcora_robust_params params;
  int updates = 0;
  std::vector<PoseMeas> meas;
  std::vector<char> update;
  std::vector<char> meas_zero;
  RobustEdges edges;
  bool ranked = false;
  std::vector<int> edge_ids;
  DevBuf<double> X_initial;
  std::vector<HostCsr> Qpat, Cpat;
  HostCsr central_pat;
};

class RbcdSession : public ExchangeSession {
 public:
  int d = 0, r = 0, n = 0, R = 1;
  Partition P;
  dcora_rbcd_options opt{};
  hipStream_t st = nullptr;
  ManiDesc mg{};
  std::vector<AgentDev> agents;
  std::unique_ptr<DeviceProblem> central;
  DevBuf<double> Xg, Vg, Yg, XPrevg;
  DevBuf<int> col_start;
  DevBuf<double> evalbuf, posenorm, eval_split;
  DevBuf<int> pose_start;
  EvalOut *eval_host = nullptr;
  double *x_stage = nullptr;
  EvalOut *eval_dev = nullptr;
  int eval_seq = 0;
  DeviceProblem *last_solver = nullptr;
  double gamma = 0, alpha = 0;
  int iteration = 0;
  dcora_ropt_result last{};
  int last_result(dcora_ropt_result *res);
  double setup_ms = 0;

  ~RbcdSession();
  int init(const HostDataset &ds, const dcora_rbcd_options &o);
  std::unique_ptr<RobustSession> robust;
  int init_robust(const HostDataset &ds, const dcora_rbcd_options &o, const dcora_robust_params &p, const int *fixed,
                  bool ranked = false);
  int update_weights(bool reset_to_initial, int counts[3]);
  int compute_weights(double *shared_w, std::vector<double> *w, double counts[3]);
  int apply_weights(const std::vector<double> &w, bool reset_to_initial);
  int set_weights(const double *w);
  int get_weights(double *w) const;
  int set_X(const double *Xh);
  int get_X(double *Xh);
  int set_acceleration(bool on);
  int phase_nonselected(int selected);
  int phase_selected(int selected);
  int evaluate_central(double *cost2, double *gradnorm, double *block_norms, int *next_selected);
  int phase_evaluate_dev(double *out_dev);
  int iterate(int selected, double *cost2, double *gradnorm, double *block_norms, int *next_selected);
  int iterate_set(const int *set, int count, int allow_adjacent);
  int agent_iterate(int agent, bool do_optimization);
  int agent_get_X(int agent, double *Xh);
  int agent_set_X(int agent, const double *Xh);
  int agent_update_neighbor(int agent, int neighbor, int count, const int *frames, const double *poses, bool aux);
  std::vector<int> agent_it;
  int agent_colours(int *colours, int *ncolours) const;
  int pack_public(int agent, double *packed_dev);
  int unpack_public(int agent, const double *packed_dev);

  int x_num_agents() const override { return R; }
  int x_rank_r() const override { return r; }
  long x_num_cols() const override { return (long)(d + 1) * n; }
  int x_rank() const override { return opt.rank; }
  int x_world() const override { return opt.world_size; }
  int x_device() const override { return opt.device; }
  hipStream_t x_stream() const override { return st; }
  double *x_mirror() override { return Xg.p; }
  XAgentView x_agent(int a) const override {
    const AgentDev &ag = agents[(size_t)a];
    XAgentView v;
    v.hosted = ag.hosted;
    v.ncols = (int)ag.public_poses.size() * (d + 1);
    v.cols_dev = ag.public_cols.p;
    v.neighbors = &ag.neighbors;
    return v;
  }
  int x_phase_nonselected(int selected) override { return phase_nonselected(selected); }
  int x_phase_selected(int selected) override { return phase_selected(selected); }
  int x_phase_evaluate_dev(double *out_dev) override { return phase_evaluate_dev(out_dev); }
  int x_iterate_set(const int *set, int count, int allow_adjacent) override { return iterate_set(set, count, allow_adjacent); }
  int x_set_X(const double *Xh) override { return set_X(Xh); }
  int x_stage_hosted(double *host_area) override;

 private:
  bool restart_now() const { return opt.acceleration && ((iteration + 1) % opt.restart_interval == 0); }
  void advance_sequences();
  bool seq_advanced_ = false;
  int staged_selected_ = -1;
  int staged_iteration_ = -1;
  bool own_stream_ = true;
  bool pending_reset_ = false;
  std::vector<char> set_marks_;
  int update_nonselected_agent(AgentDev &a, bool restart);
  int update_selected_agent(AgentDev &a, bool restart);
  hipEvent_t fork_ev_ = nullptr;
  int solve_block(AgentDev &a, std::string *err, bool serial = false);
  struct MeasSplit;
  struct Assembly {
    std::vector<int> ids;
    std::vector<HostCsr> Q, C;
// ... 14 lines not shown
```

### dcora_amd/csrc/rbcd.hip

```cpp
#include "rbcd.h"
#include "env.h"
#include "host_threads.h"

#include <algorithm>
#include <atomic>
#include <chrono>
#include <cmath>
#include <cstdlib>
#include <cstring>
#include <set>

namespace dcora {

static bool group_kernels(const ManiDesc &m) {
  return group_supported(m) && !env::generic_solver();
}

static void nesterov(hipStream_t st, const ManiDesc &m, int mode, int restart, int skip_lo, int skip_hi, double alpha,
                     double gamma, double *X, double *V, double *Y, double *XPrev, double *Yloc, Buf2 Xloc,
                     const SolverCtl *ctl) {
  if (group_kernels(m))
    launch_g_nesterov(st, m, mode, restart, skip_lo, skip_hi, alpha, gamma, X, V, Y, XPrev, Yloc, Xloc, ctl);
  else
    launch_nesterov(st, m, mode, restart & 1, skip_lo, skip_hi, alpha, gamma, X, V, Y, XPrev, Yloc, Xloc.p[0]);
// ... 764 lines not shown
    return DCORA_ERR_BAD_ARG;
  }
  DCORA_HIP(hipSetDevice(opt.device));
  const AgentDev &a = agents[agent];
  const size_t B = sizeof(double) * (size_t)r * (d + 1) * a.n;
  DCORA_HIP(hipMemcpyAsync(Xh, Xg.p + (size_t)a.col0 * r, B, hipMemcpyDeviceToHost, st));
  DCORA_HIP(hipStreamSynchronize(st));
  return DCORA_OK;
}

int RbcdSession::agent_set_X(int agent, const double *Xh) {
  staged_selected_ = -1;
  if (agent < 0 || agent >= R) {
    set_last_error("rbcd: agent out of range");
    return DCORA_ERR_BAD_ARG;
  }
  DCORA_HIP(hipSetDevice(opt.device));
  const AgentDev &a = agents[agent];
  const size_t off = (size_t)a.col0 * r;
  const size_t B = sizeof(double) * (size_t)r * (d + 1) * a.n;
  DCORA_HIP(hipMemcpyAsync(Xg.p + off, Xh, B, hipMemcpyHostToDevice, st));
  DCORA_HIP(hipMemcpyAsync(Vg.p + off, Xg.p + off, B, hipMemcpyDeviceToDevice, st));
  DCORA_HIP(hipMemcpyAsync(Yg.p + off, Xg.p + off, B, hipMemcpyDeviceToDevice, st));
  DCORA_HIP(hipMemcpyAsync(XPrevg.p + off, Xg.p + off, B, hipMemcpyDeviceToDevice, st));
  DCORA_HIP(hipStreamSynchronize(st));
  agents[agent].v_feasible = false;
  if ((int)set_marks_.size() != R) set_marks_.assign(R, 0);
  set_marks_[agent] = 1;
  bool all = true;
  for (int q = 0; q < R; ++q) all = all && (set_marks_[q] || !agents[q].hosted);
  if (all) {
    gamma = alpha = 0;
    iteration = 0;
    seq_advanced_ = false;
    pending_reset_ = false;
    agent_it.assign(R, 0);
    set_marks_.assign(R, 0);
  }
  return DCORA_OK;
}

int RbcdSession::evaluate_central(double *cost2, double *gradnorm, double *block_norms, int *next_selected) {
  if (!central) {
    set_last_error("central evaluation needs world_size == 1");
    return DCORA_ERR_UNSUPPORTED;
  }
  DeviceProblem &c = *central;
  const bool gf = c.group && c.fused && !c.has_bsr && c.Q.n_long == 0;
  const bool gfb = c.group && c.has_bsr;
  if (!gf && !gfb) c.enqueue_egrad(Xg.p, c.EG0.p, c.pA.p);
  if (c.group) {
    int nA = c.npA();
    int wpa = 0;
    if (gf)
      nA = launch_fused_grad(st, c.m, c.Q.view(), buf1(Xg.p), nullptr, buf1(c.EG0.p), buf1(c.RG0.p),
                             Buf2{{nullptr, nullptr}}, 0, c.pA.p, c.pB.p, posenorm.p, Gate{});
    else if (gfb)
      nA = launch_fused_grad_bsr(st, c.m.r, c.m.d, c.Qb.view(), buf1(Xg.p), nullptr, Buf2{{nullptr, nullptr}},
                                 Buf2{{nullptr, nullptr}}, Buf2{{nullptr, nullptr}}, 0, c.pA.p, c.pB.p, posenorm.p,
                                 Gate{}, pose_start.p, R, &wpa);
    else
      c.enq_rgrad(buf1(Xg.p), buf1(c.EG0.p), buf1(c.RG0.p), Buf2{{nullptr, nullptr}}, 0, c.pB.p, Gate{}, posenorm.p);
    const int want = ++eval_seq;
    launch_eval_finish(st, R, pose_start.p, posenorm.p, c.pA.p, nA, eval_dev, want, eval_split.p, n,
                       wpa > 0 ? c.pB.p : nullptr, wpa);
    const auto t0 = std::chrono::steady_clock::now();
    unsigned spins = 0;
    while (eval_host->seq != want) {
      if ((++spins & 4095u) == 0 &&
          std::chrono::duration<double>(std::chrono::steady_clock::now() - t0).count() > 20.0) {
        set_last_error("rbcd: evaluation epilogue did not complete (spin timeout)");
        return DCORA_ERR_HIP;
      }
    }
    std::atomic_thread_fence(std::memory_order_acquire);
    if (block_norms)
      for (int b = 0; b < R; ++b) block_norms[b] = eval_host->block_norms[b];
    if (cost2) *cost2 = eval_host->cost2;
    if (gradnorm) *gradnorm = eval_host->gradnorm;
    if (next_selected) *next_selected = eval_host->next;
    return DCORA_OK;
  }
  launch_rgrad(st, mg, buf1(Xg.p), buf1(c.EG0.p), buf1(c.RG0.p), Buf2{{nullptr, nullptr}}, 0, c.pB.p, Gate{});
  launch_block_dots(st, r, R, col_start.p, c.RG0.p, nullptr, evalbuf.p);
  launch_sum_partials(st, c.pA.p, c.npA(), 2, 2, evalbuf.p + 2 * R);
  std::vector<double> h(2 * R + 2);
  DCORA_HIP(hipMemcpyAsync(h.data(), evalbuf.p, sizeof(double) * (2 * R + 2), hipMemcpyDeviceToHost, st));
  DCORA_HIP(hipStreamSynchronize(st));
  double g2 = 0, best = -1;
  int arg = 0;
  for (int b = 0; b < R; ++b) {
    const double nb = std::sqrt(h[2 * b]);
    if (block_norms) block_norms[b] = nb;
    g2 += h[2 * b];
    if (nb > best) {
      best = nb;
      arg = b;
    }
  }
  if (cost2) *cost2 = 2.0 * (0.5 * h[2 * R] + h[2 * R + 1]);
  if (gradnorm) *gradnorm = std::sqrt(g2);
  if (next_selected) *next_selected = arg;
  return DCORA_OK;
}

int RbcdSession::last_result(dcora_ropt_result *res) {
  if (last_solver) return last_solver->fetch_result(res);
  *res = last;
  return DCORA_OK;
}

int RbcdSession::phase_evaluate_dev(double *out_dev) {
  DCORA_HIP(hipSetDevice(opt.device));
  DCORA_HIP(hipMemsetAsync(out_dev, 0, sizeof(double) * 2 * R, st));
  for (AgentDev &a : agents) {
    if (!a.hosted) continue;
    DeviceProblem &pb = *a.prob;
    const double *Xb = Xg.p + (size_t)a.col0 * r;
// ... 173 lines not shown
```

### dcora_amd/csrc/solver_fused.hip

```cpp
#include <algorithm>
#include <stdexcept>
#include <atomic>
#include <type_traits>
#include <vector>
#include <cstdlib>
#include <cstring>

#include "kernels.h"
#include "tcg_rules.h"

namespace dcora {

namespace {

constexpr int GW = 8;

__device__ __forceinline__ double f_partial4_load(const double *__restrict__ p, int np) {
  const int l = (int)(threadIdx.x & 63u);
  const double a = (l < np) ? p[l] : 0.0, b = (l + 64 < np) ? p[l + 64] : 0.0;
  const double c = (l + 128 < np) ? p[l + 128] : 0.0, d = (l + 192 < np) ? p[l + 192] : 0.0;
  return (a + b) + (c + d);
}
__device__ __forceinline__ int f_partial_index(int np) { return np <= 64 ? (int)(threadIdx.x & 63u) : (int)threadIdx.x; }
__device__ __forceinline__ double f_partial_total(double v, int np, double *sm) {
  return np <= 64 ? wave_sum(v) : block_sum(v, sm);
}
__device__ __forceinline__ double grp_sum(double v) {
  asm volatile("" : "+v"(v));
  v += dpp_move<0xB1>(v);
  asm volatile("" : "+v"(v));
  v += dpp_move<0x4E>(v);
  asm volatile("" : "+v"(v));
  v += dpp_move<0x141>(v);
  return v;
}

template <int D>
struct Row {
  double e[D + 1];
};
template <int D>
__device__ __forceinline__ void ld_row(const double *__restrict__ p, int r, int t, bool active, Row<D> &R) {
#pragma unroll
  for (int a = 0; a <= D; ++a) R.e[a] = active ? p[a * r + t] : 0.0;
}
template <int D>
__device__ __forceinline__ void st_row(double *__restrict__ p, int r, int t, bool active, const Row<D> &R) {
  if (active)
#pragma unroll
    for (int a = 0; a <= D; ++a) p[a * r + t] = R.e[a];
}
template <int D>
__device__ __forceinline__ void grp_sym_gram(const Row<D> &Y, const Row<D> &E, double (&S)[D][D]) {
#pragma unroll
  for (int a = 0; a < D; ++a)
#pragma unroll
    for (int b = a; b < D; ++b) {
      const double s = grp_sum(0.5 * (Y.e[a] * E.e[b] + Y.e[b] * E.e[a]));
      S[a][b] = s;
      S[b][a] = s;
    }
// ... 258 lines not shown
  double acc = 0;
#pragma unroll
  for (int q = 0; q < GB; ++q) acc += gw[q] * (beta * ga[q] - gz[q]);
  for (int base = pbeg; base < pend; base += kHessTile) {
    const int cnt = min(kHessTile, pend - base);
    if (base != pbeg) {
      __syncthreads();
      for (int i = threadIdx.x; i < cnt; i += kBlock) {
        s_ci[i] = Q.ci[base + i];
        s_v[i] = Q.v[base + i];
      }
      __syncthreads();
    }
    int lo = max(myb, base) - base;
    const int hi = min(mye, base + cnt) - base;
    if (base == pbeg) lo += GB;
    for (int p = lo; p < hi; p += 8) {
      double a8[8], b8[8], w8[8];
#pragma unroll
      for (int q = 0; q < 8; ++q) {
        const bool ok = p + q < hi;
        const size_t oo = ok ? (size_t)s_ci[p + q] * r + t : 0;
        w8[q] = ok ? s_v[p + q] : 0.0;
        b8[q] = z[oo];
        a8[q] = (iter > 0) ? d_old[oo] : 0.0;
      }
#pragma unroll
      for (int q = 0; q < 8; ++q) acc += w8[q] * (beta * a8[q] - b8[q]);
    }
  }
  if (act) {
    const double dn = (iter > 0) ? beta * d_own - z_own : -z_own;
    d_new[oown] = dn;
    s_W[e] = acc;
    s_D[e] = dn;
  }
  __syncthreads();
  Row<D> V, W;
#pragma unroll
  for (int a = 0; a < DH; ++a) {
    W.e[a] = pact ? s_W[(g * DH + a) * r + tt] : 0.0;
    V.e[a] = pact ? s_D[(g * DH + a) * r + tt] : 0.0;
  }
  row_sub_AS<D>(W, V, S);
  row_tangent<D>(Y, W);
  st_row<D>(Hd + o, r, tt, pact, W);
  double dacc = 0;
#pragma unroll
  for (int a = 0; a < DH; ++a) dacc += V.e[a] * W.e[a];
  const double tot = block_sum(dacc, s_red);
  if (threadIdx.x == 0) p1[blockIdx.x] = tot;
}

template <int D>
__global__ __launch_bounds__(kBlock) void k_fused_grad(ManiDesc m, CsrDev Q, Buf2 Xb, const double *__restrict__ G,
                                                       Buf2 EGb, Buf2 RGb, Buf2 Sb, int sel,
                                                       double *__restrict__ pA, double *__restrict__ pB,
                                                       double *__restrict__ posenorm, Gate g) {
  if (gated(g.ctl, g.seq, g.gate)) return;
  __shared__ int s_ci[kHessTile];
  __shared__ double s_v[kHessTile];
  __shared__ double s_W[kBlock], s_X[kBlock];
  __shared__ double s_red[16];
  constexpr int DH = D + 1;
  const int idx = g.ctl ? ((g.ctl->cur ^ sel) & 1) : 0;
  const double *__restrict__ X = Xb.p[idx];
  double *__restrict__ EG = EGb.p[idx];
  double *__restrict__ RG = RGb.p[idx];
  double *__restrict__ Sblk = Sb.p[idx];
  const int r = m.r;
  const int PB = fused_pb(r, DH);
  const int pose0 = blockIdx.x * PB;
  const int npose = min(PB, m.n - pose0);
  const int j0 = pose0 * DH, ncol = npose * DH, nout = ncol * r;
  const int e = threadIdx.x;
  const bool act = e < nout;
  const int lc = e / r, t = e - lc * r;
  const int j = j0 + lc;
  const int pbeg = Q.rp[j0], pend = Q.rp[j0 + ncol];
  const int myb = act ? Q.rp[j] : 0, mye = act ? Q.rp[j + 1] : 0;
  const size_t oown = (size_t)j * r + t;
  const double x_own = act ? X[oown] : 0.0;
  const double g_own = (act && G) ? G[oown] : 0.0;
  double acc = 0;
  for (int base = pbeg; base < pend; base += kHessTile) {
    const int cnt = min(kHessTile, pend - base);
    if (base != pbeg) __syncthreads();
    {
      constexpr int SU = kHessTile / kBlock;
      int ci_r[SU];
      double v_r[SU];
      const int last = max(pend - 1, 0);
#pragma unroll
      for (int u = 0; u < SU; ++u) {
        const int i = min(base + (int)threadIdx.x + u * kBlock, last);
        ci_r[u] = Q.ci[i];
        v_r[u] = Q.v[i];
      }
#pragma unroll
      for (int u = 0; u < SU; ++u) {
        const int i = threadIdx.x + u * kBlock;
        if (i < cnt) {
          s_ci[i] = ci_r[u];
          s_v[i] = v_r[u];
        }
      }
    }
    __syncthreads();
    const int lo = max(myb, base) - base, hi = min(mye, base + cnt) - base;
    for (int p = lo; p < hi; p += 8) {
      double b8[8], w8[8];
#pragma unroll
      for (int q = 0; q < 8; ++q) {
        const bool ok = p + q < hi;
        const size_t oo = ok ? (size_t)s_ci[p + q] * r + t : 0;
        w8[q] = ok ? s_v[p + q] : 0.0;
        b8[q] = X[oo];
      }
#pragma unroll
      for (int q = 0; q < 8; ++q) acc += w8[q] * b8[q];
    }
  }
  double d0 = 0, d1 = 0;
  if (act) {
    const double eg = acc + g_own;
    EG[oown] = eg;
    s_W[e] = eg;
    s_X[e] = x_own;
    d0 = acc * x_own;
    d1 = x_own * g_own;
  }
  __syncthreads();
  const int gp = threadIdx.x >> 3, tt = threadIdx.x & (GW - 1);
  const bool pact = (gp < npose) && (tt < r);
  const int pose = pose0 + gp;
  const size_t o = (size_t)pose * DH * r;
  Row<D> Y, E;
#pragma unroll
  for (int a = 0; a < DH; ++a) {
    E.e[a] = pact ? s_W[(gp * DH + a) * r + tt] : 0.0;
    Y.e[a] = pact ? s_X[(gp * DH + a) * r + tt] : 0.0;
  }
  double S[D][D];
  grp_sym_gram<D>(Y, E, S);
  if (Sblk && gp < npose && tt == 0)
#pragma unroll
    for (int a = 0; a < D; ++a)
#pragma unroll
      for (int b = 0; b < D; ++b) Sblk[(size_t)pose * D * D + a + b * D] = S[a][b];
  row_sub_AS<D>(E, Y, S);
  double pa = 0;
#pragma unroll
  for (int a = 0; a < DH; ++a) pa += E.e[a] * E.e[a];
  if (posenorm) {
    const double ps = grp_sum(pa);
    if (gp < npose && tt == 0) posenorm[pose] = ps;
  }
  st_row<D>(RG + o, r, tt, pact, E);
  const double t0 = block_sum(d0, s_red);
  const double t1 = block_sum(d1, s_red);
  const double t2 = block_sum(pact ? pa : 0.0, s_red);
  if (threadIdx.x == 0) {
    pA[2 * blockIdx.x] = t0;
    pA[2 * blockIdx.x + 1] = t1;
    pB[blockIdx.x] = t2;
  }
}

template <int D>
__global__ __launch_bounds__(kBlock) void k_fused_hess_bsr(ManiDesc m, BsrDev A, const double *__restrict__ z,
                                                           const double *__restrict__ d_old,
                                                           double *__restrict__ d_new, Buf2 Xb, Buf2 Sb,
                                                           double *__restrict__ Hd, const double *__restrict__ p3,
                                                           int np3, double *__restrict__ p1, SolverCtl *ctl, int seq,
                                                           int iter) {
  const int par = iter & 1;
  const int st_o = ctl->outer_done_stamp, st_t = ctl->tcg_done_stamp, cur = ctl->cur & 1;
  const double c_zr = ctl->z_r[par ^ 1], c_alpha = ctl->alpha, c_dPd = ctl->d_Pd[par ^ 1], c_ePd = ctl->e_Pd[par ^ 1],
               c_ePen = ctl->e_Pe_n;
  constexpr int DH = D + 1, BS = DH * DH;
  __shared__ double s_bv[kBsrTile * BS];
  __shared__ int s_bc[kBsrTile];
  __shared__ double s_red[16];
  const int r = m.r;
  const int pose0 = blockIdx.x * kPosesPerBlock;
  const int g = threadIdx.x >> 3, tt = threadIdx.x & (GW - 1);
  const int pose = pose0 + g;
  const bool inr = pose < m.n;
  const bool pact = inr && (tt < r);
  const size_t o = (size_t)pose * DH * r;
  const int pi3 = f_partial_index(np3);
  double myp = (pi3 < np3) ? p3[pi3] : 0.0;
  const int pend_pose = min(m.n, pose0 + kPosesPerBlock);
  const int bbeg = A.bp[pose0], bend = A.bp[pend_pose];
  const int myb = inr ? A.bp[pose] : 0, mye = inr ? A.bp[pose + 1] : 0;
  Row<D> Zo, Do, Y;
  ld_row<D>(z + o, r, tt, pact, Zo);
  if (iter > 0) {
    ld_row<D>(d_old + o, r, tt, pact, Do);
  } else {
#pragma unroll
    for (int a = 0; a < DH; ++a) Do.e[a] = 0.0;
  }
  const double *__restrict__ X = Xb.p[cur];
  const double *__restrict__ Sblk = Sb.p[cur];
  ld_row<D>(X + o, r, tt, pact, Y);
  double S[D][D];
#pragma unroll
  for (int a = 0; a < D; ++a)
#pragma unroll
    for (int b = 0; b < D; ++b) S[a][b] = inr ? Sblk[(size_t)pose * D * D + a + b * D] : 0.0;
  for (int i = threadIdx.x + kBlock; i < np3; i += kBlock) myp += p3[i];
  if (seq > st_o || seq > st_t) return;
  const double z_r_new = f_partial_total(myp, np3, s_red);
  double beta = 0;
  if (iter > 0) beta = tcg_beta(z_r_new, c_zr);
  if (blockIdx.x == 0 && threadIdx.x == 0) {
    if (iter == 0)
// ... 1468 lines not shown
      for (int i = 0; i < R; ++i) pa += e[i] * e[i];
      if (!active) pa = 0;
      dg += pa;
      if (go.posenorm) {
        const double ps = quad_sum(pa);
        if (inr && c == 0) go.posenorm[pose] = ps;
      }
      if (RG) st_run<R>(RG + oc, active, e);
    }
  }
  if (DOTS) {
    const double a = block_sum(d0, s_red);
    const double b = block_sum(d1, s_red);
    if (threadIdx.x == 0) {
      partials[2 * blockIdx.x] = a;
      partials[2 * blockIdx.x + 1] = b;
    }
  }
  if (GRAD) {
    const double cs = block_sum(dg, s_red);
    if (threadIdx.x == 0) go.pB[blockIdx.x] = cs;
  }
}


int group_grid(int n) {
  long g = ((long)n + kPosesPerBlock - 1) / kPosesPerBlock;
  if (g < 1) g = 1;
  if (g > kMaxPartials) g = kMaxPartials;
  return (int)g;
}

}

__global__ void k_ctl_init(SolverCtl *c, double tol, double Delta, double maxDelta, int max_outer, int stop_on_accept,
                           int max_inner) {
  if (threadIdx.x != 0 || blockIdx.x != 0) return;
  c->f1 = c->ngf = c->fInit = c->gradNormInit = 0;
  CtlInit ci;
  ci.tol = tol;
  ci.Delta = Delta;
  ci.maxDelta = maxDelta;
  ci.max_outer = max_outer;
  ci.stop_on_accept = stop_on_accept;
  ci.max_inner = max_inner;
  ctl_arm(c, ci);
}
void launch_ctl_init(hipStream_t st, SolverCtl *c, double tol, double Delta, double maxDelta, int max_outer,
                     int stop_on_accept, int max_inner) {
  hipLaunchKernelGGL(k_ctl_init, dim3(1), dim3(64), 0, st, c, tol, Delta, maxDelta, max_outer, stop_on_accept,
                     max_inner);
}

constexpr int kEvalSplit = 32;
__global__ __launch_bounds__(kBlock) void k_eval_partial(const int *__restrict__ pose_start,
                                                         const double *__restrict__ posenorm,
                                                         double *__restrict__ part) {
  __shared__ double s_red[16];
  const int b = blockIdx.x / kEvalSplit, sl = blockIdx.x - b * kEvalSplit;
  const int lo = pose_start[b], hi = pose_start[b + 1];
  const int per = (hi - lo + kEvalSplit - 1) / kEvalSplit;
  const int i0 = lo + sl * per, i1 = min(hi, i0 + per);
  double v = 0;
  for (int i = i0 + (int)threadIdx.x; i < i1; i += kBlock) v += posenorm[i];
  v = block_sum(v, s_red);
  if (threadIdx.x == 0) part[blockIdx.x] = v;
}
__global__ __launch_bounds__(kBlock) void k_eval_finish(int R, const int *__restrict__ pose_start,
                                                        const double *__restrict__ posenorm,
                                                        const double *__restrict__ pA, int npA, EvalOut *out,
                                                        int seq, const double *__restrict__ part,
                                                        const double *__restrict__ agent_partials, int wpa) {
  __shared__ double s_red[16];
  __shared__ double s_bn[kMaxAgents];
  double q0 = ((int)threadIdx.x < npA) ? pA[2 * threadIdx.x] : 0.0;
  double q1 = ((int)threadIdx.x < npA) ? pA[2 * threadIdx.x + 1] : 0.0;
  if (agent_partials) {
    const int w = threadIdx.x >> 6, lane = threadIdx.x & 63, nw = kBlock / 64;
    for (int b = w; b < R; b += nw) {
      const int lo = b * wpa, hi = lo + wpa;
      double v = 0;
      for (int i0 = lo + lane; i0 < hi; i0 += 64 * 8) {
        double t8[8];
#pragma unroll
        for (int u = 0; u < 8; ++u) t8[u] = agent_partials[min(i0 + 64 * u, hi - 1)];
#pragma unroll
        for (int u = 0; u < 8; ++u) v += (i0 + 64 * u < hi) ? t8[u] : 0.0;
      }
      v = wave_sum(v);
      if (lane == 0) s_bn[b] = v;
    }
  } else if (part) {
    if ((int)threadIdx.x < R) {
      double v = 0;
      for (int u = 0; u < kEvalSplit; ++u) v += part[threadIdx.x * kEvalSplit + u];
      s_bn[threadIdx.x] = v;
    }
  } else
  {
    const int w = threadIdx.x >> 6, lane = threadIdx.x & 63, nw = kBlock / 64;
    for (int b = w; b < R; b += nw) {
      const int lo = pose_start[b], hi = pose_start[b + 1];
      double v = 0;
      for (int i0 = lo + lane; i0 < hi; i0 += 64 * 8) {
        double t8[8];
#pragma unroll
        for (int u = 0; u < 8; ++u) t8[u] = posenorm[min(i0 + 64 * u, hi - 1)];
#pragma unroll
        for (int u = 0; u < 8; ++u) v += (i0 + 64 * u < hi) ? t8[u] : 0.0;
      }
      v = wave_sum(v);
      if (lane == 0) s_bn[b] = v;
    }
  }
  for (int i0 = threadIdx.x + kBlock; i0 < npA; i0 += 8 * kBlock) {
    double a8[8], c8[8];
#pragma unroll
    for (int u = 0; u < 8; ++u) {
      const int i = i0 + u * kBlock;
      a8[u] = i < npA ? pA[2 * i] : 0.0;
      c8[u] = i < npA ? pA[2 * i + 1] : 0.0;
    }
#pragma unroll
    for (int u = 0; u < 8; ++u) {
      q0 += a8[u];
      q1 += c8[u];
    }
  }
  const double fq = block_sum(q0, s_red);
  const double fg = block_sum(q1, s_red);
  if (threadIdx.x == 0) {
    double g2 = 0, best = -1;
    int arg = 0;
    for (int b = 0; b < R; ++b) {
      const double nb = sqrt(s_bn[b]);
      out->block_norms[b] = nb;
      g2 += s_bn[b];
      if (nb > best) {
        best = nb;
        arg = b;
      }
    }
    out->cost2 = 2.0 * (0.5 * fq + fg);
    out->gradnorm = sqrt(g2);
    out->next = arg;
    __threadfence_system();
    __hip_atomic_store(const_cast<int *>(&out->seq), seq, __ATOMIC_RELEASE, __HIP_MEMORY_SCOPE_SYSTEM);
  }
}
void launch_eval_finish(hipStream_t st, int R, const int *pose_start, const double *posenorm, const double *pA,
                        int npA, EvalOut *out_dev, int seq, double *split_scratch, int nposes,
                        const double *agent_partials, int wg_per_agent) {
  const bool split = !agent_partials && split_scratch && nposes >= 16384;
  if (split)
    hipLaunchKernelGGL(k_eval_partial, dim3(R * kEvalSplit), dim3(kBlock), 0, st, pose_start, posenorm, split_scratch);
  hipLaunchKernelGGL(k_eval_finish, dim3(1), dim3(kBlock), 0, st, R, pose_start, posenorm, pA, npA, out_dev, seq,
                     split ? split_scratch : nullptr, agent_partials, wg_per_agent);
}
int eval_split_doubles() { return kMaxAgents * kEvalSplit; }

int spmm_bsr_grid(int nbrows) {
  const int cap = kBsrMaxGrid, per = kPosesPerBlock;
  long g = ((long)nbrows + per - 1) / per;
  if (g < 1) g = 1;
  if (g > cap) g = cap;
  return (int)g;
}
template <bool DOTS, bool GRAD>
static bool launch_bsrq(hipStream_t st, int grid, int r, int d, const BsrDev &A, Buf2 X, int selX, const double *G, Buf2 Y,
                        int selY, double *partials, Gate g, const BsrGradOut &go) {
#define DCORA_BSRQ(D_, R_)                                                                                              \
  if (d == D_ && r == R_) {                                                                                             \
    hipLaunchKernelGGL((k_spmm_bsrq<D_, R_, DOTS, GRAD>), dim3(grid), dim3(kQBlock), 0, st, A, X, selX, G, Y, selY, \
                       partials, g, go);                                                                                \
    return true;                                                                                                        \
  }
  DCORA_BSRQ(3, 3) DCORA_BSRQ(3, 4) DCORA_BSRQ(3, 5) DCORA_BSRQ(3, 6) DCORA_BSRQ(3, 7) DCORA_BSRQ(3, 8)
  DCORA_BSRQ(2, 2) DCORA_BSRQ(2, 3) DCORA_BSRQ(2, 4) DCORA_BSRQ(2, 5) DCORA_BSRQ(2, 6) DCORA_BSRQ(2, 7) DCORA_BSRQ(2, 8)
#undef DCORA_BSRQ
  return false;
}
void launch_spmm_bsr(hipStream_t st, int r, int d, const BsrDev &A, Buf2 X, int selX, const double *G, Buf2 Y,
                     int selY, double *partials, Gate g) {
  const int grid = spmm_bsr_grid(A.nbrows);
  const BsrGradOut none{};
  const bool ok = partials ? launch_bsrq<true, false>(st, grid, r, d, A, X, selX, G, Y, selY, partials, g, none)
                           : launch_bsrq<false, false>(st, grid, r, d, A, X, selX, G, Y, selY, partials, g, none);
  if (!ok) throw std::logic_error("block Q-apply: no instantiation for this (d, r); the block structure is built for d <= r <= 8 only");
}
int launch_fused_grad_bsr(hipStream_t st, int r, int d, const BsrDev &A, Buf2 X, const double *G, Buf2 EG, Buf2 RG, Buf2 S,
                          int sel, double *pA, double *pB, double *posenorm, Gate g, const int *agent_start, int agents,
                          int *wg_per_agent) {
  int grid = spmm_bsr_grid(A.nbrows);
  BsrGradOut go;
  go.RG = RG;
  go.S = S;
  go.pB = pB;
  go.posenorm = posenorm;
  if (agent_start && agents > 0 && wg_per_agent) {
    const int wpa = std::max(1, grid / agents);
    grid = wpa * agents;
// ... 223 lines not shown
      }
      for (int i = 0; i < 64; ++i) buf[i] = 0;
      if (n == 500) {
        fprintf(stderr, "k_tcg_run stamps (us from start, workgroup 0, mean of %d runs with >= 4 iterations):", n);
        for (int i = 0; i < 34; ++i) fprintf(stderr, " %.2f", acc[i] / n);
        fprintf(stderr, "\n");
        n = -1000000;
      }
    }
    ++count;
    a.stamps = buf;
  }
#endif
  if (m.r == 4) return tcg_run_launch<4>(st, a);
  if (m.r == 5) return tcg_run_launch<5>(st, a);
  if (m.r == 6) return tcg_run_launch<6>(st, a);
  return -1;
}
int launch_fused_pc(hipStream_t st, const ManiDesc &m, int ldm, const double *Minv, Buf2 grad, Buf2 X,
                    const double *delta, const double *Hd, double *eta, double *Heta, const double *res_old,
                    double *res_new, double *z, const double *p1, int np1, double *p3, SolverCtl *ctl, HostFlags *hf,
                    int seq, int iter, int first, double *pC) {
  return fused_pc_dispatch(st, m, ldm, Minv, grad, X, delta, Hd, eta, Heta, res_old, res_new, z, p1, np1, p3, ctl, hf,
                           seq, iter, first, pC, false);
}
bool fused_pc_ready(const ManiDesc &m, int ldm) {
  Buf2 none{};
  return fused_pc_dispatch(nullptr, m, ldm, nullptr, none, none, nullptr, nullptr, nullptr, nullptr, nullptr, nullptr,
                           nullptr, nullptr, 0, nullptr, nullptr, nullptr, 0, 0, 0, nullptr, true) >= 0;
}
void launch_fused_finish(hipStream_t st, const ManiDesc &m, Buf2 X, const double *Zpart, const double *res,
                         double *z, const double *p2, int np2, double *p3, SolverCtl *ctl, HostFlags *hf, int seq,
                         int iter, int first, int nsplit, SpFold sf, double *zraw) {
  const int grid = fused_pose_blocks(m);
  const int ns = nsplit > 0 ? nsplit : fused_nsplit(m);
  if (m.d == 3)
    hipLaunchKernelGGL(k_fused_finish<3>, dim3(grid), dim3(kBlock), 0, st, m, ns, X, Zpart, res, z, p2, np2, p3, ctl,
                       hf, seq, iter, first, sf, zraw);
  else
    hipLaunchKernelGGL(k_fused_finish<2>, dim3(grid), dim3(kBlock), 0, st, m, ns, X, Zpart, res, z, p2, np2, p3, ctl,
                       hf, seq, iter, first, sf, zraw);
}

int launch_g_rgrad(hipStream_t st, const ManiDesc &m, Buf2 X, Buf2 EG, Buf2 RG, Buf2 Sblk, int sel, double *partials,
                   double *posenorm, Gate g) {
  const int grid = group_grid(m.n);
  if (m.d == 3)
    hipLaunchKernelGGL(k_g_rgrad<3>, dim3(grid), dim3(kBlock), 0, st, m, X, EG, RG, Sblk, sel, partials, posenorm, g);
  else
    hipLaunchKernelGGL(k_g_rgrad<2>, dim3(grid), dim3(kBlock), 0, st, m, X, EG, RG, Sblk, sel, partials, posenorm, g);
  return grid;
}
int launch_fused_grad(hipStream_t st, const ManiDesc &m, const CsrDev &Q, Buf2 X, const double *G, Buf2 EG, Buf2 RG,
                      Buf2 Sblk, int sel, double *pA, double *pB, double *posenorm, Gate g) {
  const int grid = fused_pose_blocks(m);
  if (m.d == 3)
    hipLaunchKernelGGL(k_fused_grad<3>, dim3(grid), dim3(kBlock), 0, st, m, Q, X, G, EG, RG, Sblk, sel, pA, pB, posenorm,
                       g);
  else
    hipLaunchKernelGGL(k_fused_grad<2>, dim3(grid), dim3(kBlock), 0, st, m, Q, X, G, EG, RG, Sblk, sel, pA, pB, posenorm,
                       g);
  return grid;
}
int launch_g_retract(hipStream_t st, const ManiDesc &m, Buf2 X, const double *V, double alpha, Buf2 out, int selOut,
                     Buf2 grad, const double *HV, double *partials, Gate g) {
  const int grid = group_grid(m.n);
  if (m.d == 3)
    hipLaunchKernelGGL(k_g_retract<3>, dim3(grid), dim3(kBlock), 0, st, m, X, V, alpha, out, selOut, grad, HV,
                       partials, g);
  else
    hipLaunchKernelGGL(k_g_retract<2>, dim3(grid), dim3(kBlock), 0, st, m, X, V, alpha, out, selOut, grad, HV,
                       partials, g);
  return grid;
}
void launch_g_nesterov(hipStream_t st, const ManiDesc &m, int mode, int restart, int skip_lo, int skip_hi,
                       double alpha, double gamma, double *X, double *V, double *Y, double *XPrev, double *Yloc,
                       Buf2 Xloc, const SolverCtl *ctl, double *inner_Yloc) {
  GNesterovArgs a{mode, restart, skip_lo, skip_hi, alpha, gamma, X, V, Y, XPrev, Yloc, inner_Yloc, Xloc, ctl};
  const int grid = group_grid(m.n);
  if (m.d == 3)
    hipLaunchKernelGGL(k_g_nesterov<3>, dim3(grid), dim3(kBlock), 0, st, m, a);
  else
    hipLaunchKernelGGL(k_g_nesterov<2>, dim3(grid), dim3(kBlock), 0, st, m, a);
}

}
```

### include/dcora_hip.h

```cpp
#ifndef DCORA_HIP_H_
#define DCORA_HIP_H_

#ifdef __cplusplus
extern "C" {
#endif

typedef enum {
  DCORA_OK = 0,
  DCORA_ERR_BAD_ARG = 1,
  DCORA_ERR_NO_DEVICE = 2,
  DCORA_ERR_HIP = 3,
  DCORA_ERR_NOT_PD = 4,
  DCORA_ERR_NO_CONVERGENCE = 5,
  DCORA_ERR_NO_PRECONDITIONER = 6,
  DCORA_ERR_IO = 7,
  DCORA_ERR_UNSUPPORTED = 8,
  DCORA_ERR_EXCHANGE_LINK = 9
} dcora_status;

const char *dcora_status_string(int status);
const char *dcora_last_error(void);
int dcora_device_count(void);

enum {
// ... 82 lines not shown
int dcora_dataset_load_g2o(const char *path, dcora_dataset_t *out);
int dcora_dataset_create(int d, int n, int m, const int *ids, const double *vals, dcora_dataset_t *out);
int dcora_dataset_info(dcora_dataset_t ds, int *d, int *n, int *m);
int dcora_dataset_copy(dcora_dataset_t ds, int *ids, double *vals);
int dcora_dataset_destroy(dcora_dataset_t ds);
int dcora_dataset_chordal_init(dcora_dataset_t ds, double *T);
int dcora_dataset_chordal_init_device(dcora_dataset_t ds, int device, double *T);
int dcora_graph_build_Q_pgo(int d, int n, int agent_id, int m, const int *ids, const double *vals, dcora_csr_t *Q);

typedef struct dcora_radataset_s *dcora_radataset_t;
int dcora_radataset_load_pyfg(const char *path, dcora_radataset_t *out);
int dcora_radataset_info(dcora_radataset_t ds, int *info);
int dcora_radataset_create(int d, int n, int l, int b, int m_pp, const int *pp_ids, const double *pp_vals, int m_pl,
                           const int *pl_ids, const double *pl_vals, int m_rg, const int *rg_ids, const double *rg_vals,
                           const double *gt, dcora_radataset_t *out);
int dcora_radataset_copy(dcora_radataset_t ds, int *pp_ids, double *pp_vals, int *pl_ids, double *pl_vals, int *rg_ids,
                         double *rg_vals);
int dcora_radataset_ground_truth(dcora_radataset_t ds, double *gt);
int dcora_radataset_build_Q(dcora_radataset_t ds, dcora_csr_t *Q);
int dcora_radataset_odometry_init(dcora_radataset_t ds, unsigned long long seed, double *X0);
int dcora_radataset_ownership(dcora_radataset_t ds, int *pose_robot, int *sphere_robot, int *landmark_robot);
int dcora_radataset_agent_columns(dcora_radataset_t ds, int robot, int *dims3, int *own, int *k_a);
int dcora_graph_extract_agent_blocks(int k, const int *rowptr, const int *colidx, const double *vals, int k_a,
                                     const int *own, dcora_csr_t *Qaa, dcora_csr_t *C);
int dcora_radataset_destroy(dcora_radataset_t ds);
int dcora_graph_precond_regularization(int k, const int *rowptr, const int *colidx, const double *vals, int device,
                                       double *reg);

typedef struct dcora_rbcd_s *dcora_rbcd_t;
typedef struct {
  int num_robots;
  int r;
  int acceleration;
  int restart_interval;
  dcora_ropt_params local;
  int rank, world_size;
  int device;
  void *stream;
} dcora_rbcd_options;
void dcora_rbcd_options_default(dcora_rbcd_options *o);

int dcora_rbcd_create(dcora_dataset_t ds, const dcora_rbcd_options *opt, dcora_rbcd_t *out);
int dcora_rbcd_destroy(dcora_rbcd_t s);
int dcora_rbcd_set_X(dcora_rbcd_t s, const double *X);
int dcora_rbcd_get_X(dcora_rbcd_t s, double *X);
int dcora_rbcd_iterate(dcora_rbcd_t s, int selected, double *cost2, double *gradnorm, double *block_norms,
                       int *next_selected);
int dcora_rbcd_run(dcora_rbcd_t s, int max_iters, double rgrad_tol, int *iters_done, double *cost2_trace,
                   double *gradnorm_trace, int *selected_trace);
int dcora_rbcd_iterate_set(dcora_rbcd_t s, const int *set, int count, int allow_adjacent);
int dcora_rbcd_set_acceleration(dcora_rbcd_t s, int acceleration);
int dcora_rbcd_agent_colours(dcora_rbcd_t s, int *colours, int *ncolours);
int dcora_rbcd_evaluate(dcora_rbcd_t s, double *cost2, double *gradnorm, double *block_norms, int *next_selected);
int dcora_rbcd_agent_iterate(dcora_rbcd_t s, int agent, int do_optimization);
int dcora_rbcd_agent_update_neighbor(dcora_rbcd_t s, int agent, int neighbor, int count, const int *frames,
                                     const double *poses, int auxiliary);
int dcora_rbcd_agent_last_skipped(dcora_rbcd_t s, int agent, int *skipped);
int dcora_rbcd_agent_get_X(dcora_rbcd_t s, int agent, double *X);
int dcora_rbcd_agent_set_X(dcora_rbcd_t s, int agent, const double *X);
int dcora_rbcd_agent_info(dcora_rbcd_t s, int agent, int *num_poses, int *first_pose, int *iteration_number);
int dcora_rbcd_last_result(dcora_rbcd_t s, dcora_ropt_result *res);

int dcora_rbcd_X_device_ptr(dcora_rbcd_t s, double **X_dev);
int dcora_rbcd_public_count(dcora_rbcd_t s, int agent, int *count);
int dcora_rbcd_public_indices(dcora_rbcd_t s, int agent, int *global_pose_idx);
int dcora_rbcd_pack_public_dev(dcora_rbcd_t s, int agent, double *packed_dev);
int dcora_rbcd_unpack_public_dev(dcora_rbcd_t s, int agent, const double *packed_dev);
int dcora_rbcd_phase_nonselected(dcora_rbcd_t s, int selected);
int dcora_rbcd_phase_selected(dcora_rbcd_t s, int selected);
int dcora_rbcd_phase_evaluate_dev(dcora_rbcd_t s, double *out_dev);
int dcora_rbcd_synchronize(dcora_rbcd_t s);
int dcora_rbcd_profile_tcg_runs(dcora_rbcd_t s, int enable);
int dcora_rbcd_profile_tcg_read(dcora_rbcd_t s, double *out2);

typedef struct dcora_exchange_s *dcora_exchange_t;
int dcora_exchange_create(dcora_rbcd_t s, const char *job_name, dcora_exchange_t *out);
int dcora_exchange_destroy(dcora_exchange_t ex);
int dcora_exchange_info(dcora_exchange_t ex, double *info10);
int dcora_exchange_link_report(dcora_exchange_t ex, double *out4);
int dcora_exchange_post(dcora_exchange_t ex, const int *agents, int count);
int dcora_exchange_wait(dcora_exchange_t ex, const int *agents, int count);
int dcora_exchange_evaluate(dcora_exchange_t ex, double *cost2, double *gradnorm, double *block_norms,
                            int *next_selected);
int dcora_exchange_rbcd_iterate(dcora_exchange_t ex, int selected, double *cost2, double *gradnorm,
                                double *block_norms, int *next_selected);
int dcora_exchange_rbcd_tick(dcora_exchange_t ex, const int *set, int count, int allow_adjacent);
int dcora_exchange_set_X(dcora_exchange_t ex, const double *X);
int dcora_exchange_gather_X(dcora_exchange_t ex, double *X);
int dcora_exchange_barrier(dcora_exchange_t ex);
int dcora_exchange_all_ready(dcora_exchange_t ex, int ready, int *all_ready);
int dcora_exchange_certify(dcora_exchange_t ex, int k, const int *rowptr, const int *colidx, const double *vals,
                           double eta, int *certified, double *theta, double *lambda_min, double *v, long long *matvecs,
                           int *distributed);
int dcora_exchange_host_selftest(const char *job_name, int rank, int world_size, int num_agents, int rounds,
                                 double *checksum);
int dcora_debug_exchange_leave_stale(const char *job_name, int world_size, int num_agents);
int dcora_debug_exchange_probe_fault(int rounds);

typedef struct dcora_ra_rbcd_s *dcora_ra_rbcd_t;
int dcora_ra_rbcd_create(dcora_radataset_t ds, const dcora_rbcd_options *opt, dcora_ra_rbcd_t *out);
int dcora_exchange_create_ra(dcora_ra_rbcd_t s, const char *job_name, dcora_exchange_t *out);
int dcora_ra_rbcd_destroy(dcora_ra_rbcd_t s);
int dcora_ra_rbcd_info(dcora_ra_rbcd_t s, int *num_agents, int *robots);
int dcora_ra_rbcd_set_X(dcora_ra_rbcd_t s, const double *X);
int dcora_ra_rbcd_get_X(dcora_ra_rbcd_t s, double *X);
int dcora_ra_rbcd_iterate(dcora_ra_rbcd_t s, int selected, double *cost2, double *gradnorm, double *block_norms,
// ... 74 lines not shown
```

Baseline: 4242.

## Fold RTR init/decide and eval-finish reductions into fused-grad kernel tail

New measurement: 4263 (median of 2 runs). About the same (+0.5%).

```diff
diff --git a/dcora_amd/__init__.py b/dcora_amd/__init__.py
--- a/dcora_amd/__init__.py
+++ b/dcora_amd/__init__.py
@@ -323,7 +323,8 @@
 def _solver_info(self):
     info = np.zeros(2)
     check(capi.lib().dcora_problem_solver_info(self.h, info))
-    return {"tcg": {0: "three launches", 1: "two launches", 2: "one launch per run"}[int(info[0])]}
+    return {"tcg": {0: "three launches", 1: "two launches", 2: "one launch per run"}[int(info[0])],
+            "eval": "tail" if info[1] else "launch"}
 
 
 QuadraticProblem.solver_info = _solver_info
@@ -537,6 +538,11 @@
         col, nc = np.zeros(self.R, np.int32), C.c_int()
         check(capi.lib().dcora_rbcd_agent_colours(self.h, col, C.byref(nc)))
         return col, nc.value
+
+    def solver_info(self):
+        info = np.zeros(1)
+        check(capi.lib().dcora_rbcd_solver_info(self.h, info))
+        return {"eval": "tail" if info[0] else "launch"}
 
     def evaluate(self):
         c2, gn, nxt = C.c_double(), C.c_double(), C.c_int()
diff --git a/dcora_amd/capi.py b/dcora_amd/capi.py
--- a/dcora_amd/capi.py
+++ b/dcora_amd/capi.py
@@ -176,6 +176,7 @@
     "dcora_debug_tcg_run_fault": (C.c_int, [C.c_int]),
     "dcora_debug_tcg_run_fault_at": (C.c_int, [C.c_int, C.c_int]),
     "dcora_problem_solver_info": (C.c_int, [_vp, _dp]),
+    "dcora_rbcd_solver_info": (C.c_int, [_vp, _dp]),
     "dcora_ra_rbcd_create": (C.c_int, [_vp, C.POINTER(RbcdOptions), C.POINTER(_vp)]),
     "dcora_ra_rbcd_destroy": (C.c_int, [_vp]),
     "dcora_ra_rbcd_info": (C.c_int, [_vp, _PI, _vp]),
diff --git a/dcora_amd/csrc/capi.hip b/dcora_amd/csrc/capi.hip
--- a/dcora_amd/csrc/capi.hip
+++ b/dcora_amd/csrc/capi.hip
@@ -268,6 +268,7 @@
   return abi_call({p, info}, [&]() -> int {
     const DeviceProblem &P = p->p;
     info[0] = !P.use_pc() ? 0 : (P.tcg_run_ok ? 2 : 1);
+    info[1] = P.eval_tail ? 1 : 0;
     return DCORA_OK;
   });
 }
@@ -1049,6 +1050,12 @@
 int dcora_rbcd_evaluate(dcora_rbcd_t s, double *cost2, double *gradnorm, double *block_norms, int *next_selected) {
   return abi_call({s}, [&] { return s->s.evaluate_central(cost2, gradnorm, block_norms, next_selected); });
 }
+int dcora_rbcd_solver_info(dcora_rbcd_t s, double *info) {
+  return abi_call({s, info}, [&]() -> int {
+    info[0] = s->s.central_eval_tail() ? 1 : 0;
+    return DCORA_OK;
+  });
+}
 int dcora_rbcd_agent_iterate(dcora_rbcd_t s, int agent, int do_optimization) {
   return abi_call({s}, [&] { return s->s.agent_iterate(agent, do_optimization != 0); });
 }
diff --git a/dcora_amd/csrc/device_problem.h b/dcora_amd/csrc/device_problem.h
--- a/dcora_amd/csrc/device_problem.h
+++ b/dcora_amd/csrc/device_problem.h
@@ -206,6 +206,8 @@
   bool tcg_run_ok = false;
   bool concurrent_solves = false;
   DevBuf<unsigned> tcg_sync;
+  bool eval_tail = false;
+  DevBuf<unsigned> eval_arrive;
   bool profile_tcg_runs = false;
   std::vector<hipEvent_t> run_events;
   size_t run_events_used = 0;
diff --git a/dcora_amd/csrc/device_problem.hip b/dcora_amd/csrc/device_problem.hip
--- a/dcora_amd/csrc/device_problem.hip
+++ b/dcora_amd/csrc/device_problem.hip
@@ -241,6 +241,11 @@
     }
   }
   DCORA_HIP(ctl.alloc(1));
+  eval_tail = fused && !has_bsr && Q.n_long == 0 && !env::eval_launch();
+  if (eval_tail) {
+    DCORA_HIP(eval_arrive.alloc(1));
+    DCORA_HIP(hipMemsetAsync(eval_arrive.p, 0, sizeof(unsigned), st));
+  }
   {
     const int rc2 = host_flags_acquire(&hf, &hf_dev, &hf_slot);
     if (rc2) return rc2;
@@ -793,6 +798,7 @@
   const int nsl;
   const int nZ;
   const bool gf, gfb;
+  const bool tail;
   unsigned *const sync_p;
   const int nsync;
   double *const dbuf[2];
@@ -808,14 +814,14 @@
         folded(sparse && p.sp.foldable()), sf(folded ? p.sp.fold() : SpFold{}), nsl(sparse ? 1 : -1),
         nZ(f == TcgForm::pc || f == TcgForm::run ? fused_pc_blocks(p.m) : nPB),
         gf(f != TcgForm::generic && !p.has_bsr && p.Q.n_long == 0), gfb(f != TcgForm::generic && p.has_bsr),
-        sync_p(f == TcgForm::run ? p.tcg_sync.p : nullptr), nsync(f == TcgForm::run ? tcg_run_sync_words() : 0),
+        tail(gf && p.eval_tail), sync_p(f == TcgForm::run ? p.tcg_sync.p : nullptr), nsync(f == TcgForm::run ? tcg_run_sync_words() : 0),
         dbuf{p.delta.p, p.delta2.p}, rbuf{p.res.p, p.res2.p} {}
 
   bool outer_done() const { return p.hf->outer_done_seq >= solve_first; }
   bool stopped(int tcg_first) const { return p.hf->tcg_done_seq >= tcg_first || outer_done(); }
   int nAe() const { return gf ? nPB : nA; }
 
-  int eval(int sel) {
+  int eval(int sel, const CtlInit &ci = CtlInit(), int nR = 0) {
     const auto g = [&] {
       ++seq;
       return sel ? Gate{c, seq, 1} : Gate{};
@@ -826,7 +832,23 @@
       launch_rgrad(p.st, p.m, p.Xb(), p.EGb(), p.RGb(), p.Sb(), sel, p.pB.p, g());
       return nP;
     }
-    if (gf) return launch_fused_grad(p.st, p.m, Qv, p.Xb(), Gp, p.EGb(), p.RGb(), p.Sb(), sel, p.pA.p, p.pB.p, nullptr, g());
+    if (gf) {
+      const Gate gg = g();
+      EvalTail t;
+      if (tail) {
+        t.mode = sel ? kTailRtrDecide : kTailRtrInit;
+        t.arrive = p.eval_arrive.p;
+        t.seq = ++seq;
+        t.ctl = c;
+        t.hf = p.hf_dev;
+        t.ci = ci;
+        t.pC = p.pC.p;
+        t.npC = nR;
+        t.tcg_sync = sync_p;
+        t.nsync = nsync;
+      }
+      return launch_fused_grad(p.st, p.m, Qv, p.Xb(), Gp, p.EGb(), p.RGb(), p.Sb(), sel, p.pA.p, p.pB.p, nullptr, gg, t);
+    }
     if (gfb)
       return launch_fused_grad_bsr(p.st, p.m.r, p.m.d, Qbv, p.Xb(), Gp, kNoBuf, p.RGb(), p.Sb(), sel, p.pA.p, p.pB.p,
                                    nullptr, g());
@@ -1008,8 +1030,8 @@
   };
   auto run_gave_up = [&]() { return f.form == TcgForm::run && hf->tcg_abort_seq >= f.solve_first; };
 
-  int nG = f.eval(0);
-  launch_rtr_init(st, pA.p, f.nAe(), pB.p, nG, f.c, hf_dev, ++seq, ci, f.sync_p, f.nsync);
+  int nG = f.eval(0, ci);
+  if (!f.tail) launch_rtr_init(st, pA.p, f.nAe(), pB.p, nG, f.c, hf_dev, ++seq, ci, f.sync_p, f.nsync);
   int last_pace_seq = seq;
   std::vector<int> last_seq((size_t)std::max(1, max_inner));
   int next_first_seq = time_is_up() ? 0 : f.first();
@@ -1050,8 +1072,8 @@
       last_seq[j] = seq;
     }
     const int nR = f.trial();
-    nG = f.eval(1);
-    launch_rtr_decide(st, pA.p, f.nAe(), pB.p, nG, pC.p, nR, f.c, hf_dev, ++seq, f.sync_p, f.nsync);
+    nG = f.eval(1, CtlInit(), nR);
+    if (!f.tail) launch_rtr_decide(st, pA.p, f.nAe(), pB.p, nG, pC.p, nR, f.c, hf_dev, ++seq, f.sync_p, f.nsync);
     last_pace_seq = seq;
     if (outer + 1 < max_outer) next_first_seq = time_is_up() ? 0 : f.first();
   }
diff --git a/dcora_amd/csrc/env.cpp b/dcora_amd/csrc/env.cpp
--- a/dcora_amd/csrc/env.cpp
+++ b/dcora_amd/csrc/env.cpp
@@ -24,6 +24,9 @@
 }
 int solver_tcg() {
   return is("DCORA_SOLVER_TCG", "launch") ? -1 : is("DCORA_SOLVER_TCG", "run") ? 1 : 0;
+}
+bool eval_launch() {
+  return is("DCORA_SOLVER_EVAL", "launch");
 }
 int solver_bc() {
   static const int v = is("DCORA_SOLVER_BC", "pc") ? 1 : is("DCORA_SOLVER_BC", "split") ? -1 : 0;
diff --git a/dcora_amd/csrc/env.h b/dcora_amd/csrc/env.h
--- a/dcora_amd/csrc/env.h
+++ b/dcora_amd/csrc/env.h
@@ -7,6 +7,7 @@
 int precond_mode();
 bool generic_solver();
 int solver_tcg();
+bool eval_launch();
 int solver_bc();
 bool factor_on_host();
 bool fill_on_host();
diff --git a/dcora_amd/csrc/eval_tail.h b/dcora_amd/csrc/eval_tail.h
--- /dev/null
+++ b/dcora_amd/csrc/eval_tail.h
@@ -0,0 +1,229 @@
+#pragma once
+#include "kernels.h"
+#include "tcg_rules.h"
+
+namespace dcora {
+
+template <bool HANDOFF>
+__device__ __forceinline__ double ld_handoff(const double *p) {
+  if constexpr (HANDOFF)
+    return __hip_atomic_load(const_cast<double *>(p), __ATOMIC_RELAXED, __HIP_MEMORY_SCOPE_AGENT);
+  else
+    return *p;
+}
+template <bool HANDOFF>
+__device__ __forceinline__ void st_handoff(double *p, double v) {
+  if constexpr (HANDOFF)
+    __hip_atomic_store(p, v, __ATOMIC_RELAXED, __HIP_MEMORY_SCOPE_AGENT);
+  else
+    *p = v;
+}
+
+__device__ __forceinline__ bool tail_arrive(unsigned *arrive, int *s_flag) {
+  asm volatile("s_waitcnt vmcnt(0)" ::: "memory");
+  __syncthreads();
+  if (threadIdx.x == 0) {
+    const unsigned ticket = __hip_atomic_fetch_add(arrive, 1u, __ATOMIC_RELAXED, __HIP_MEMORY_SCOPE_AGENT);
+    const bool last = ticket == gridDim.x - 1;
+    if (last) __hip_atomic_store(arrive, 0u, __ATOMIC_RELAXED, __HIP_MEMORY_SCOPE_AGENT);
+    *s_flag = last ? 1 : 0;
+  }
+  __syncthreads();
+  const bool last = *s_flag != 0;
+  __builtin_amdgcn_fence(__ATOMIC_ACQUIRE, "wavefront");
+  return last;
+}
+
+template <int N, bool HANDOFF>
+__device__ __forceinline__ void sum_partials_n(const double *const (&p)[N], const int (&np)[N], const int (&st)[N],
+                                               const int (&off)[N], double *sm, double (&out)[N]) {
+  double v[N];
+#pragma unroll
+  for (int q = 0; q < N; ++q)
+    v[q] = ld_handoff<HANDOFF>(p[q] + (size_t)max(min((int)threadIdx.x, np[q] - 1), 0) * st[q] + off[q]);
+#pragma unroll
+  for (int q = 0; q < N; ++q) v[q] = ((int)threadIdx.x < np[q]) ? v[q] : 0.0;
+#pragma unroll
+  for (int q = 0; q < N; ++q)
+    for (int i = threadIdx.x + blockDim.x; i < np[q]; i += blockDim.x)
+      v[q] += ld_handoff<HANDOFF>(p[q] + (size_t)i * st[q] + off[q]);
+#pragma unroll
+  for (int q = 0; q < N; ++q) v[q] = wave_sum(v[q]);
+  const int w = threadIdx.x >> 6, nw = (blockDim.x + 63) >> 6;
+  __syncthreads();
+  if ((threadIdx.x & 63) == 0)
+#pragma unroll
+    for (int q = 0; q < N; ++q) sm[q * 4 + w] = v[q];
+  __syncthreads();
+#pragma unroll
+  for (int q = 0; q < N; ++q) {
+    double t = 0;
+    for (int i = 0; i < nw; ++i) t += sm[q * 4 + i];
+    out[q] = t;
+  }
+}
+
+template <bool HANDOFF>
+__device__ __forceinline__ void rtr_init_body(const double *pA, int npA, const double *pB, int npB, SolverCtl *ctl,
+                                              HostFlags *hf, int seq, const CtlInit &ci, unsigned *tcg_sync, int nsync,
+                                              double *s_red) {
+  for (int i = threadIdx.x; i < nsync; i += kBlock) tcg_sync[i] = 0u;
+  if (ci.enable && threadIdx.x == 0) ctl_arm(ctl, ci);
+  const double *const ps[3] = {pA, pA, pB};
+  const int nps[3] = {npA, npA, npB}, sts[3] = {2, 2, 1}, offs[3] = {0, 1, 0};
+  double sums[3];
+  sum_partials_n<3, HANDOFF>(ps, nps, sts, offs, s_red, sums);
+  const double fq = sums[0], fg = sums[1], g2 = sums[2];
+  if (threadIdx.x == 0) {
+    ctl->f1 = 0.5 * fq + fg;
+    ctl->ngf = sqrt(g2);
+    ctl->fInit = ctl->f1;
+    ctl->gradNormInit = ctl->ngf;
+    if (ctl->ngf < ctl->tol || ctl->max_outer <= 0) {
+      ctl->outer_done_stamp = seq;
+      host_store(&hf->outer_done_seq, seq);
+    }
+    host_store(&hf->last_seq_done, seq);
+  }
+}
+
+template <bool HANDOFF>
+__device__ __forceinline__ void rtr_decide_body(const double *pA, int npA, const double *pB, int npB,
+                                                const double *pC, int npC, SolverCtl *ctl, HostFlags *hf, int seq,
+                                                unsigned *tcg_sync, int nsync, double *s_red) {
+  for (int i = threadIdx.x; i < nsync; i += kBlock) tcg_sync[i] = 0u;
+  const double c_f1 = ctl->f1, c_ngf = ctl->ngf, c_Delta = ctl->Delta, c_maxDelta = ctl->maxDelta, c_tol = ctl->tol;
+  const int c_status = ctl->tcg_status, c_cur = ctl->cur, c_accepted = ctl->accepted, c_outer_it = ctl->outer_it,
+            c_max_outer = ctl->max_outer, c_stop_on_accept = ctl->stop_on_accept;
+  const double *const ps[5] = {pA, pA, pB, pC, pC};
+  const int nps[5] = {npA, npA, npB, npC, npC}, sts[5] = {2, 2, 1, 2, 2}, offs[5] = {0, 1, 0, 0, 1};
+  double sums[5];
+  sum_partials_n<5, HANDOFF>(ps, nps, sts, offs, s_red, sums);
+  const double fq = sums[0], fg = sums[1], g2 = sums[2], eg = sums[3], eh = sums[4];
+  if (threadIdx.x == 0) {
+    const double f2 = 0.5 * fq + fg;
+    const double rho = (c_f1 - f2) / (-(eg + 0.5 * eh));
+    ctl->f2 = f2;
+    ctl->rho = rho;
+    if (rho > 0.75) {
+      if (c_status == TR_NEGCURVTURE || c_status == TR_EXCREGION) ctl->Delta = fmin(2.0 * c_Delta, c_maxDelta);
+    } else if (rho < 0.25) {
+      ctl->Delta = c_Delta * 0.25;
+    }
+    const bool accept = (rho > 0.1) && isfinite(rho);
+    double ngf = c_ngf;
+    if (accept) {
+      ngf = sqrt(g2);
+      ctl->cur = c_cur ^ 1;
+      ctl->f1 = f2;
+      ctl->ngf = ngf;
+      ctl->accepted = c_accepted + 1;
+      ctl->last_accepted = 1;
+    } else {
+      ctl->last_accepted = 0;
+      host_store(&hf->reject_seq, seq);
+    }
+    ctl->outer_it = c_outer_it + 1;
+    if (ngf < c_tol || c_outer_it + 1 >= c_max_outer || (c_stop_on_accept && accept)) {
+      ctl->outer_done_stamp = seq;
+      host_store(&hf->outer_done_seq, seq);
+    }
+    host_store(&hf->last_seq_done, seq);
+  }
+}
+
+constexpr int kEvalSplit = 32;
+template <bool HANDOFF>
+__device__ __forceinline__ void eval_finish_body(int R, const int *__restrict__ pose_start, const double *posenorm,
+                                                 const double *pA, int npA, EvalOut *out, int seq, const double *part,
+                                                 const double *agent_partials, int wpa, double *s_red, double *s_bn) {
+  const int iq = max(min((int)threadIdx.x, npA - 1), 0);
+  double q0 = ld_handoff<HANDOFF>(pA + 2 * iq);
+  double q1 = ld_handoff<HANDOFF>(pA + 2 * iq + 1);
+  q0 = ((int)threadIdx.x < npA) ? q0 : 0.0;
+  q1 = ((int)threadIdx.x < npA) ? q1 : 0.0;
+  if (agent_partials) {
+    const int w = threadIdx.x >> 6, lane = threadIdx.x & 63, nw = kBlock / 64;
+    for (int b = w; b < R; b += nw) {
+      const int lo = b * wpa, hi = lo + wpa;
+      double v = 0;
+      for (int i0 = lo + lane; i0 < hi; i0 += 64 * 8) {
+        double t8[8];
+#pragma unroll
+        for (int u = 0; u < 8; ++u) t8[u] = ld_handoff<HANDOFF>(agent_partials + min(i0 + 64 * u, hi - 1));
+#pragma unroll
+        for (int u = 0; u < 8; ++u) v += (i0 + 64 * u < hi) ? t8[u] : 0.0;
+      }
+      v = wave_sum(v);
+      if (lane == 0) s_bn[b] = v;
+    }
+  } else if (part) {
+    if ((int)threadIdx.x < R) {
+      double v = 0;
+      for (int u = 0; u < kEvalSplit; ++u) v += ld_handoff<HANDOFF>(part + threadIdx.x * kEvalSplit + u);
+      s_bn[threadIdx.x] = v;
+    }
+  } else
+  {
+    const int w = threadIdx.x >> 6, lane = threadIdx.x & 63, nw = kBlock / 64;
+    for (int b = w; b < R; b += nw) {
+      const int lo = pose_start[b], hi = pose_start[b + 1];
+      double v = 0;
+      for (int i0 = lo + lane; i0 < hi; i0 += 64 * 8) {
+        double t8[8];
+#pragma unroll
+        for (int u = 0; u < 8; ++u) t8[u] = ld_handoff<HANDOFF>(posenorm + min(i0 + 64 * u, hi - 1));
+#pragma unroll
+        for (int u = 0; u < 8; ++u) v += (i0 + 64 * u < hi) ? t8[u] : 0.0;
+      }
+      v = wave_sum(v);
+      if (lane == 0) s_bn[b] = v;
+    }
+  }
+  for (int i0 = threadIdx.x + kBlock; i0 < npA; i0 += 8 * kBlock) {
+    double a8[8], c8[8];
+#pragma unroll
+    for (int u = 0; u < 8; ++u) {
+      const int i = i0 + u * kBlock;
+      a8[u] = i < npA ? ld_handoff<HANDOFF>(pA + 2 * i) : 0.0;
+      c8[u] = i < npA ? ld_handoff<HANDOFF>(pA + 2 * i + 1) : 0.0;
+    }
+#pragma unroll
+    for (int u = 0; u < 8; ++u) {
+      q0 += a8[u];
+      q1 += c8[u];
+    }
+  }
+  const double fq = block_sum(q0, s_red);
+  const double fg = block_sum(q1, s_red);
+  if (threadIdx.x == 0) {
+    double g2 = 0, best = -1;
+    int arg = 0;
+    for (int b = 0; b < R; ++b) {
+      const double nb = sqrt(s_bn[b]);
+      out->block_norms[b] = nb;
+      g2 += s_bn[b];
+      if (nb > best) {
+        best = nb;
+        arg = b;
+      }
+    }
+    out->cost2 = 2.0 * (0.5 * fq + fg);
+    out->gradnorm = sqrt(g2);
+    out->next = arg;
+    __threadfence_system();
+    __hip_atomic_store(const_cast<int *>(&out->seq), seq, __ATOMIC_RELEASE, __HIP_MEMORY_SCOPE_SYSTEM);
+  }
+}
+
+__device__ __forceinline__ void eval_tail_run(const EvalTail &t, const double *pA, int npA, const double *pB, int npB,
+                                              const double *posenorm, double *s_red, double *s_bn) {
+  if (t.mode == kTailRtrInit)
+    rtr_init_body<true>(pA, npA, pB, npB, t.ctl, t.hf, t.seq, t.ci, t.tcg_sync, t.nsync, s_red);
+  else if (t.mode == kTailRtrDecide)
+    rtr_decide_body<true>(pA, npA, pB, npB, t.pC, t.npC, t.ctl, t.hf, t.seq, t.tcg_sync, t.nsync, s_red);
+  else if (t.mode == kTailEvalFinish)
+    eval_finish_body<true>(t.R, t.pose_start, posenorm, pA, npA, t.out, t.seq, nullptr, nullptr, 0, s_red, s_bn);
+}
+
+}
diff --git a/dcora_amd/csrc/kernels.h b/dcora_amd/csrc/kernels.h
--- a/dcora_amd/csrc/kernels.h
+++ b/dcora_amd/csrc/kernels.h
@@ -137,6 +137,22 @@
   int enable = 0;
   double tol = 0, Delta = 0, maxDelta = 0;
   int max_outer = 0, stop_on_accept = 0, max_inner = 0;
+};
+enum EvalTailMode : int { kTailNone = 0, kTailRtrInit = 1, kTailRtrDecide = 2, kTailEvalFinish = 3 };
+struct EvalTail {
+  int mode = kTailNone;
+  unsigned *arrive = nullptr;
+  int seq = 0;
+  SolverCtl *ctl = nullptr;
+  HostFlags *hf = nullptr;
+  CtlInit ci;
+  const double *pC = nullptr;
+  int npC = 0;
+  unsigned *tcg_sync = nullptr;
+  int nsync = 0;
+  int R = 0;
+  const int *pose_start = nullptr;
+  EvalOut *out = nullptr;
 };
 void launch_rtr_init(hipStream_t st, const double *pA, int npA, const double *pB, int npB, SolverCtl *ctl,
                      HostFlags *hf, int seq, CtlInit ci = CtlInit(), unsigned *tcg_sync = nullptr, int nsync = 0);
@@ -209,7 +225,8 @@
                           int sel, double *pA, double *pB, double *posenorm, Gate g,
                           const int *agent_start = nullptr, int agents = 0, int *wg_per_agent = nullptr);
 int launch_fused_grad(hipStream_t st, const ManiDesc &m, const CsrDev &Q, Buf2 X, const double *G, Buf2 EG, Buf2 RG,
-                      Buf2 Sblk, int sel, double *pA, double *pB, double *posenorm, Gate g);
+                      Buf2 Sblk, int sel, double *pA, double *pB, double *posenorm, Gate g,
+                      const EvalTail &tail = EvalTail() );
 int launch_g_rgrad(hipStream_t st, const ManiDesc &m, Buf2 X, Buf2 EG, Buf2 RG, Buf2 Sblk, int sel, double *partials,
                    double *posenorm, Gate g);
 void launch_ctl_init(hipStream_t st, SolverCtl *c, double tol, double Delta, double maxDelta, int max_outer,
diff --git a/dcora_amd/csrc/kernels.hip b/dcora_amd/csrc/kernels.hip
--- a/dcora_amd/csrc/kernels.hip
+++ b/dcora_amd/csrc/kernels.hip
@@ -1,32 +1,8 @@
 #include "kernels.h"
+#include "eval_tail.h"
 #include "tcg_rules.h"
 
 namespace dcora {
-
-template <int N>
-__device__ __forceinline__ void sum_partials_n(const double *const (&p)[N], const int (&np)[N], const int (&st)[N],
-                                               const int (&off)[N], double *sm, double (&out)[N]) {
-  double v[N];
-#pragma unroll
-  for (int q = 0; q < N; ++q) v[q] = ((int)threadIdx.x < np[q]) ? p[q][(size_t)threadIdx.x * st[q] + off[q]] : 0.0;
-#pragma unroll
-  for (int q = 0; q < N; ++q)
-    for (int i = threadIdx.x + blockDim.x; i < np[q]; i += blockDim.x) v[q] += p[q][(size_t)i * st[q] + off[q]];
-#pragma unroll
-  for (int q = 0; q < N; ++q) v[q] = wave_sum(v[q]);
-  const int w = threadIdx.x >> 6, nw = (blockDim.x + 63) >> 6;
-  __syncthreads();
-  if ((threadIdx.x & 63) == 0)
-#pragma unroll
-    for (int q = 0; q < N; ++q) sm[q * 4 + w] = v[q];
-  __syncthreads();
-#pragma unroll
-  for (int q = 0; q < N; ++q) {
-    double t = 0;
-    for (int i = 0; i < nw; ++i) t += sm[q * 4 + i];
-    out[q] = t;
-  }
-}
 
 int vec_grid(long nelem) {
   long g = (nelem + kBlock - 1) / kBlock;
@@ -1398,24 +1374,7 @@
                                                      SolverCtl *ctl, HostFlags *hf, int seq, CtlInit ci,
                                                      unsigned *tcg_sync, int nsync) {
   __shared__ double s_red[16];
-  for (int i = threadIdx.x; i < nsync; i += kBlock) tcg_sync[i] = 0u;
-  if (ci.enable && threadIdx.x == 0) ctl_arm(ctl, ci);
-  const double *const ps[3] = {pA, pA, pB};
-  const int nps[3] = {npA, npA, npB}, sts[3] = {2, 2, 1}, offs[3] = {0, 1, 0};
-  double sums[3];
-  sum_partials_n<3>(ps, nps, sts, offs, s_red, sums);
-  const double fq = sums[0], fg = sums[1], g2 = sums[2];
-  if (threadIdx.x == 0) {
-    ctl->f1 = 0.5 * fq + fg;
-    ctl->ngf = sqrt(g2);
-    ctl->fInit = ctl->f1;
-    ctl->gradNormInit = ctl->ngf;
-    if (ctl->ngf < ctl->tol || ctl->max_outer <= 0) {
-      ctl->outer_done_stamp = seq;
-      host_store(&hf->outer_done_seq, seq);
-    }
-    host_store(&hf->last_seq_done, seq);
-  }
+  rtr_init_body<false>(pA, npA, pB, npB, ctl, hf, seq, ci, tcg_sync, nsync, s_red);
 }
 
 __global__ __launch_bounds__(kBlock) void k_tcg_begin(long nelem, Buf2 gradb, double *__restrict__ eta,
@@ -1521,40 +1480,7 @@
                                                        int seq, unsigned *tcg_sync, int nsync) {
   if (gated(ctl, seq, 1)) return;
   __shared__ double s_red[20];
-  for (int i = threadIdx.x; i < nsync; i += kBlock) tcg_sync[i] = 0u;
-  const double *const ps[5] = {pA, pA, pB, pC, pC};
-  const int nps[5] = {npA, npA, npB, npC, npC}, sts[5] = {2, 2, 1, 2, 2}, offs[5] = {0, 1, 0, 0, 1};
-  double sums[5];
-  sum_partials_n<5>(ps, nps, sts, offs, s_red, sums);
-  const double fq = sums[0], fg = sums[1], g2 = sums[2], eg = sums[3], eh = sums[4];
-  if (threadIdx.x == 0) {
-    const double f2 = 0.5 * fq + fg;
-    const double rho = (ctl->f1 - f2) / (-(eg + 0.5 * eh));
-    ctl->f2 = f2;
-    ctl->rho = rho;
-    if (rho > 0.75) {
-      if (ctl->tcg_status == TR_NEGCURVTURE || ctl->tcg_status == TR_EXCREGION) ctl->Delta = fmin(2.0 * ctl->Delta, ctl->maxDelta);
-    } else if (rho < 0.25) {
-      ctl->Delta *= 0.25;
-    }
-    const bool accept = (rho > 0.1) && isfinite(rho);
-    if (accept) {
-      ctl->cur ^= 1;
-      ctl->f1 = f2;
-      ctl->ngf = sqrt(g2);
-      ctl->accepted += 1;
-      ctl->last_accepted = 1;
-    } else {
-      ctl->last_accepted = 0;
-      host_store(&hf->reject_seq, seq);
-    }
-    ctl->outer_it += 1;
-    if (ctl->ngf < ctl->tol || ctl->outer_it >= ctl->max_outer || (ctl->stop_on_accept && accept)) {
-      ctl->outer_done_stamp = seq;
-      host_store(&hf->outer_done_seq, seq);
-    }
-    host_store(&hf->last_seq_done, seq);
-  }
+  rtr_decide_body<false>(pA, npA, pB, npB, pC, npC, ctl, hf, seq, tcg_sync, nsync, s_red);
 }
 
 void launch_rtr_init(hipStream_t st, const double *pA, int npA, const double *pB, int npB, SolverCtl *ctl,
diff --git a/dcora_amd/csrc/rbcd.h b/dcora_amd/csrc/rbcd.h
--- a/dcora_amd/csrc/rbcd.h
+++ b/dcora_amd/csrc/rbcd.h
@@ -87,6 +87,10 @@
   int phase_nonselected(int selected);
   int phase_selected(int selected);
   int evaluate_central(double *cost2, double *gradnorm, double *block_norms, int *next_selected);
+  bool central_eval_tail() const {
+    return central && central->group && central->fused && !central->has_bsr && central->Q.n_long == 0 &&
+           central->eval_tail;
+  }
   int phase_evaluate_dev(double *out_dev);
   int iterate(int selected, double *cost2, double *gradnorm, double *block_norms, int *next_selected);
   int iterate_set(const int *set, int count, int allow_adjacent);
diff --git a/dcora_amd/csrc/rbcd.hip b/dcora_amd/csrc/rbcd.hip
--- a/dcora_amd/csrc/rbcd.hip
+++ b/dcora_amd/csrc/rbcd.hip
@@ -840,18 +840,29 @@
   if (c.group) {
     int nA = c.npA();
     int wpa = 0;
-    if (gf)
+    const int want = ++eval_seq;
+    const bool tail = central_eval_tail();
+    if (gf) {
+      EvalTail t;
+      if (tail) {
+        t.mode = kTailEvalFinish;
+        t.arrive = c.eval_arrive.p;
+        t.seq = want;
+        t.R = R;
+        t.pose_start = pose_start.p;
+        t.out = eval_dev;
+      }
       nA = launch_fused_grad(st, c.m, c.Q.view(), buf1(Xg.p), nullptr, buf1(c.EG0.p), buf1(c.RG0.p),
-                             Buf2{{nullptr, nullptr}}, 0, c.pA.p, c.pB.p, posenorm.p, Gate{});
-    else if (gfb)
+                             Buf2{{nullptr, nullptr}}, 0, c.pA.p, c.pB.p, posenorm.p, Gate{}, t);
+    } else if (gfb)
       nA = launch_fused_grad_bsr(st, c.m.r, c.m.d, c.Qb.view(), buf1(Xg.p), nullptr, Buf2{{nullptr, nullptr}},
                                  Buf2{{nullptr, nullptr}}, Buf2{{nullptr, nullptr}}, 0, c.pA.p, c.pB.p, posenorm.p,
                                  Gate{}, pose_start.p, R, &wpa);
     else
       c.enq_rgrad(buf1(Xg.p), buf1(c.EG0.p), buf1(c.RG0.p), Buf2{{nullptr, nullptr}}, 0, c.pB.p, Gate{}, posenorm.p);
-    const int want = ++eval_seq;
-    launch_eval_finish(st, R, pose_start.p, posenorm.p, c.pA.p, nA, eval_dev, want, eval_split.p, n,
-                       wpa > 0 ? c.pB.p : nullptr, wpa);
+    if (!tail)
+      launch_eval_finish(st, R, pose_start.p, posenorm.p, c.pA.p, nA, eval_dev, want, eval_split.p, n,
+                         wpa > 0 ? c.pB.p : nullptr, wpa);
     const auto t0 = std::chrono::steady_clock::now();
     unsigned spins = 0;
     while (eval_host->seq != want) {
diff --git a/dcora_amd/csrc/solver_fused.hip b/dcora_amd/csrc/solver_fused.hip
--- a/dcora_amd/csrc/solver_fused.hip
+++ b/dcora_amd/csrc/solver_fused.hip
@@ -7,6 +7,7 @@
 #include <cstring>
 
 #include "kernels.h"
+#include "eval_tail.h"
 #include "tcg_rules.h"
 
 namespace dcora {
@@ -371,11 +372,10 @@
   if (threadIdx.x == 0) p1[blockIdx.x] = tot;
 }
 
-template <int D>
+template <int D, bool TAIL>
 __global__ __launch_bounds__(kBlock) void k_fused_grad(ManiDesc m, CsrDev Q, Buf2 Xb, const double *__restrict__ G,
-                                                       Buf2 EGb, Buf2 RGb, Buf2 Sb, int sel,
-                                                       double *__restrict__ pA, double *__restrict__ pB,
-                                                       double *__restrict__ posenorm, Gate g) {
+                                                       Buf2 EGb, Buf2 RGb, Buf2 Sb, int sel, double *pA, double *pB,
+                                                       double *posenorm, Gate g, EvalTail tl) {
   if (gated(g.ctl, g.seq, g.gate)) return;
   __shared__ int s_ci[kHessTile];
   __shared__ double s_v[kHessTile];
@@ -473,16 +473,20 @@
   for (int a = 0; a < DH; ++a) pa += E.e[a] * E.e[a];
   if (posenorm) {
     const double ps = grp_sum(pa);
-    if (gp < npose && tt == 0) posenorm[pose] = ps;
+    if (gp < npose && tt == 0) st_handoff<TAIL>(posenorm + pose, ps);
   }
   st_row<D>(RG + o, r, tt, pact, E);
   const double t0 = block_sum(d0, s_red);
   const double t1 = block_sum(d1, s_red);
   const double t2 = block_sum(pact ? pa : 0.0, s_red);
   if (threadIdx.x == 0) {
-    pA[2 * blockIdx.x] = t0;
-    pA[2 * blockIdx.x + 1] = t1;
-    pB[blockIdx.x] = t2;
+    st_handoff<TAIL>(pA + 2 * blockIdx.x, t0);
+    st_handoff<TAIL>(pA + 2 * blockIdx.x + 1, t1);
+    st_handoff<TAIL>(pB + blockIdx.x, t2);
+  }
+  if constexpr (TAIL) {
+    if (!tail_arrive(tl.arrive, s_ci)) return;
+    eval_tail_run(tl, pA, gridDim.x, pB, gridDim.x, posenorm, s_W, s_X);
   }
 }
 
@@ -2057,7 +2061,6 @@
                      max_inner);
 }
 
-constexpr int kEvalSplit = 32;
 __global__ __launch_bounds__(kBlock) void k_eval_partial(const int *__restrict__ pose_start,
                                                          const double *__restrict__ posenorm,
                                                          double *__restrict__ part) {
@@ -2078,80 +2081,7 @@
                                                         const double *__restrict__ agent_partials, int wpa) {
   __shared__ double s_red[16];
   __shared__ double s_bn[kMaxAgents];
-  double q0 = ((int)threadIdx.x < npA) ? pA[2 * threadIdx.x] : 0.0;
-  double q1 = ((int)threadIdx.x < npA) ? pA[2 * threadIdx.x + 1] : 0.0;
-  if (agent_partials) {
-    const int w = threadIdx.x >> 6, lane = threadIdx.x & 63, nw = kBlock / 64;
-    for (int b = w; b < R; b += nw) {
-      const int lo = b * wpa, hi = lo + wpa;
-      double v = 0;
-      for (int i0 = lo + lane; i0 < hi; i0 += 64 * 8) {
-        double t8[8];
-#pragma unroll
-        for (int u = 0; u < 8; ++u) t8[u] = agent_partials[min(i0 + 64 * u, hi - 1)];
-#pragma unroll
-        for (int u = 0; u < 8; ++u) v += (i0 + 64 * u < hi) ? t8[u] : 0.0;
-      }
-      v = wave_sum(v);
-      if (lane == 0) s_bn[b] = v;
-    }
-  } else if (part) {
-    if ((int)threadIdx.x < R) {
-      double v = 0;
-      for (int u = 0; u < kEvalSplit; ++u) v += part[threadIdx.x * kEvalSplit + u];
-      s_bn[threadIdx.x] = v;
-    }
-  } else
-  {
-    const int w = threadIdx.x >> 6, lane = threadIdx.x & 63, nw = kBlock / 64;
-    for (int b = w; b < R; b += nw) {
-      const int lo = pose_start[b], hi = pose_start[b + 1];
-      double v = 0;
-      for (int i0 = lo + lane; i0 < hi; i0 += 64 * 8) {
-        double t8[8];
-#pragma unroll
-        for (int u = 0; u < 8; ++u) t8[u] = posenorm[min(i0 + 64 * u, hi - 1)];
-#pragma unroll
-        for (int u = 0; u < 8; ++u) v += (i0 + 64 * u < hi) ? t8[u] : 0.0;
-      }
-      v = wave_sum(v);
-      if (lane == 0) s_bn[b] = v;
-    }
-  }
-  for (int i0 = threadIdx.x + kBlock; i0 < npA; i0 += 8 * kBlock) {
-    double a8[8], c8[8];
-#pragma unroll
-    for (int u = 0; u < 8; ++u) {
-      const int i = i0 + u * kBlock;
-      a8[u] = i < npA ? pA[2 * i] : 0.0;
-      c8[u] = i < npA ? pA[2 * i + 1] : 0.0;
-    }
-#pragma unroll
-    for (int u = 0; u < 8; ++u) {
-      q0 += a8[u];
-      q1 += c8[u];
-    }
-  }
-  const double fq = block_sum(q0, s_red);
-  const double fg = block_sum(q1, s_red);
-  if (threadIdx.x == 0) {
-    double g2 = 0, best = -1;
-    int arg = 0;
-    for (int b = 0; b < R; ++b) {
-      const double nb = sqrt(s_bn[b]);
-      out->block_norms[b] = nb;
-      g2 += s_bn[b];
-      if (nb > best) {
-        best = nb;
-        arg = b;
-      }
-    }
-    out->cost2 = 2.0 * (0.5 * fq + fg);
-    out->gradnorm = sqrt(g2);
-    out->next = arg;
-    __threadfence_system();
-    __hip_atomic_store(const_cast<int *>(&out->seq), seq, __ATOMIC_RELEASE, __HIP_MEMORY_SCOPE_SYSTEM);
-  }
+  eval_finish_body<false>(R, pose_start, posenorm, pA, npA, out, seq, part, agent_partials, wpa, s_red, s_bn);
 }
 void launch_eval_finish(hipStream_t st, int R, const int *pose_start, const double *posenorm, const double *pA,
                         int npA, EvalOut *out_dev, int seq, double *split_scratch, int nposes,
@@ -2481,14 +2411,21 @@
   return grid;
 }
 int launch_fused_grad(hipStream_t st, const ManiDesc &m, const CsrDev &Q, Buf2 X, const double *G, Buf2 EG, Buf2 RG,
-                      Buf2 Sblk, int sel, double *pA, double *pB, double *posenorm, Gate g) {
+                      Buf2 Sblk, int sel, double *pA, double *pB, double *posenorm, Gate g, const EvalTail &tail) {
   const int grid = fused_pose_blocks(m);
-  if (m.d == 3)
-    hipLaunchKernelGGL(k_fused_grad<3>, dim3(grid), dim3(kBlock), 0, st, m, Q, X, G, EG, RG, Sblk, sel, pA, pB, posenorm,
-                       g);
+  const bool t = tail.mode != kTailNone;
+  if (m.d == 3 && t)
+    hipLaunchKernelGGL((k_fused_grad<3, true>), dim3(grid), dim3(kBlock), 0, st, m, Q, X, G, EG, RG, Sblk, sel, pA, pB,
+                       posenorm, g, tail);
+  else if (m.d == 3)
+    hipLaunchKernelGGL((k_fused_grad<3, false>), dim3(grid), dim3(kBlock), 0, st, m, Q, X, G, EG, RG, Sblk, sel, pA, pB,
+                       posenorm, g, tail);
+  else if (t)
+    hipLaunchKernelGGL((k_fused_grad<2, true>), dim3(grid), dim3(kBlock), 0, st, m, Q, X, G, EG, RG, Sblk, sel, pA, pB,
+                       posenorm, g, tail);
   else
-    hipLaunchKernelGGL(k_fused_grad<2>, dim3(grid), dim3(kBlock), 0, st, m, Q, X, G, EG, RG, Sblk, sel, pA, pB, posenorm,
-                       g);
+    hipLaunchKernelGGL((k_fused_grad<2, false>), dim3(grid), dim3(kBlock), 0, st, m, Q, X, G, EG, RG, Sblk, sel, pA, pB,
+                       posenorm, g, tail);
   return grid;
 }
 int launch_g_retract(hipStream_t st, const ManiDesc &m, Buf2 X, const double *V, double alpha, Buf2 out, int selOut,
diff --git a/include/dcora_hip.h b/include/dcora_hip.h
--- a/include/dcora_hip.h
+++ b/include/dcora_hip.h
@@ -158,6 +158,7 @@
 int dcora_rbcd_set_acceleration(dcora_rbcd_t s, int acceleration);
 int dcora_rbcd_agent_colours(dcora_rbcd_t s, int *colours, int *ncolours);
 int dcora_rbcd_evaluate(dcora_rbcd_t s, double *cost2, double *gradnorm, double *block_norms, int *next_selected);
+int dcora_rbcd_solver_info(dcora_rbcd_t s, double *info);
 int dcora_rbcd_agent_iterate(dcora_rbcd_t s, int agent, int do_optimization);
 int dcora_rbcd_agent_update_neighbor(dcora_rbcd_t s, int agent, int neighbor, int count, const int *frames,
                                      const double *poses, int auxiliary);
```
